# PacificBiosciences/aardvark

Hardware: NVIDIA B200
Metric: variant_clusters_per_sec (higher is better)
Workload: dtype int32

## Files before the change

### aardvark_b200/csrc/avk_lib.cu

```cuda
#include <cuda_runtime.h>

#include <algorithm>
#include <cstdio>
#include <cstdlib>
#include <cstring>
#include <string>
#include <chrono>
#include <thread>
#include <vector>

#include <cub/device/device_radix_sort.cuh>
#include <cub/device/device_scan.cuh>
#include <cub/device/device_select.cuh>
#include <thrust/iterator/counting_iterator.h>

#include "avk_solver.cuh"
#include "avk_thread_solver.cuh"
#include "avk_writers.h"
#include "avk_vcf.cuh"
#include "avk_inflate.cuh"

using namespace avk;

#define CK(call)                                                                                   \
    do {                                                                                           \
        cudaError_t e_ = (call);                                                                   \
        if (e_ != cudaSuccess) {                                                                   \
            ctx->err = std::string(#call) + ": " + cudaGetErrorString(e_);                         \
            return (e_ == cudaErrorMemoryAllocation) ? AVK_ERR_OOM : AVK_ERR_CUDA;                 \
        }                                                                                          \
    } while (0)


template <bool SMEM>
__device__ __forceinline__ void flush_work(typename Mem<SMEM>::addr hdr, unsigned long long *out) {
    typedef Mem<SMEM> M;
    if (lane_id() == 0 && out) {
        const u64 cells = LD64(hdr + WK_CELLS), matched = LD64(hdr + WK_MATCHED);
        const u32 al = LD32(hdr + WK_ALIGN), sp = LD32(hdr + WK_SPOPS), xp = LD32(hdr + WK_XPOPS);
        if (al) atomicAdd(out + 0, (unsigned long long)al);
        if (cells) atomicAdd(out + 1, (unsigned long long)cells);
        if (matched) atomicAdd(out + 2, (unsigned long long)matched);
        if (sp) atomicAdd(out + 3, (unsigned long long)sp);
        if (xp) atomicAdd(out + 4, (unsigned long long)xp);
    }
}
template <bool SMEM>
__device__ __forceinline__ void clear_work(typename Mem<SMEM>::addr hdr) {
    typedef Mem<SMEM> M;
    const int lane = lane_id();
    if (lane < 10) ST32(hdr + 8 + 4 * lane, 0);
    __syncwarp();
}

__device__ __forceinline__ VSeq<false> plain_seq(const u8 *p, int n) {
    VSeq<false> v;
    v.data = (u64)(uintptr_t)p; v.tail = v.data + (u64)n; v.mlen = n; v.len = n;
    return v;
}

__global__ void __launch_bounds__(256) k_alt_ed(DevBatch b, u64 v_base, u64 n_variants, u32 *alt_ed, u8 *scratch, int scratch_ints,
                                                unsigned long long *work_out) {
    const int lane = lane_id();
    const u64 warp = ((u64)blockIdx.x * blockDim.x + threadIdx.x) >> 5;
    const u64 n_warps = ((u64)gridDim.x * blockDim.x) >> 5;
    const u64 hdr = (u64)(uintptr_t)(scratch + warp * ((u64)scratch_ints * 4 + ARENA_HDR));
    clear_work<false>(hdr);
    for (u64 base = v_base + warp * 32; base < v_base + n_variants; base += n_warps * 32) {
        const u64 v = base + lane;
        bool coop = false;
        if (v < v_base + n_variants) {
            const u32 l0 = b.l0[v], l1 = b.l1[v];
            if (l0 == 1 && l1 == 1) alt_ed[v] = (b.pool[b.aoff[v]] != b.pool[b.aoff[v] + 1]) ? 1u : 0u;
            else coop = true;
        }
        unsigned m = __ballot_sync(AVK_FULL, coop);
        while (m) {
            const int src = __ffs(m) - 1;
            m &= m - 1;
            const u64 vv = base + src;
            const int l0 = (int)b.l0[vv], l1 = (int)b.l1[vv];
            const u8 *a0 = b.pool + b.aoff[vv];
            const u8 *a1 = a0 + l0;
            int ed;
            const int mn = min(l0, l1);
            if (mn == 0) ed = max(l0, l1);
            else if (2 * max(l0, l1) + 3 > scratch_ints) ed = 0;
            else {
                const int p = raw_lcp<false>((u64)(uintptr_t)a0, (u64)(uintptr_t)a1, mn);
                if (p == mn) ed = max(l0, l1) - mn;
                else {
                    ed = wfa_ed_warp<false>(plain_seq(a0, l0), plain_seq(a1, l1), hdr + ARENA_HDR, (scratch_ints - 3) / 2, hdr);
                    if (ed < 0) ed = 0;
                }
            }
            if (lane == 0) alt_ed[vv] = (u32)ed;
        }
    }
    flush_work<false>(hdr, work_out);
}

__global__ void __launch_bounds__(256) k_wfa_ed(const u32 *list, const u32 *n_list, const u8 *pool, const u64 *a_off, const u32 *a_len,
                                                const u64 *b_off, const u32 *b_len, u32 *ed_out, u8 *scratch,
                                                int scratch_ints, u32 *counter, unsigned long long *work_out) {
    const int lane = lane_id();
    const u64 warp = ((u64)blockIdx.x * blockDim.x + threadIdx.x) >> 5;
    const u64 hdr = (u64)(uintptr_t)(scratch + warp * ((u64)scratch_ints * 4 + ARENA_HDR));
    clear_work<false>(hdr);
    const u32 n_pairs = *n_list;
    for (;;) {
        u32 p = 0;
        if (lane == 0) p = atomicAdd(counter, 1u);
        p = __shfl_sync(AVK_FULL, p, 0);
        if (p >= n_pairs) break;
        p = list[p];
        const int ed = wfa_ed_warp<false>(plain_seq(pool + a_off[p], (int)a_len[p]), plain_seq(pool + b_off[p], (int)b_len[p]),
                                          hdr + ARENA_HDR, (scratch_ints - 3) / 2, hdr);
        if (lane == 0) ed_out[p] = (u32)ed;
    }
    flush_work<false>(hdr, work_out);
}

__global__ void __launch_bounds__(COOP_THREADS, 1) k_wfa_ed_cta(const u32 *list, const u32 *n_list, const u8 *pool, const u64 *a_off, const u32 *a_len,
                                                                const u64 *b_off, const u32 *b_len, u32 *ed_out, u8 *scratch, int scratch_ints,
                                                                int cap_ints, u32 *counter, unsigned long long *work_out) {
    __shared__ u32 s_idx;
    CoopJob &J = *(CoopJob *)avk_dyn_smem;
    const u64 hdr = (u64)(uintptr_t)(scratch + (u64)blockIdx.x * ((u64)scratch_ints * 4 + ARENA_HDR));
    if (threadIdx.x < 32) clear_work<false>(hdr);
    const u32 n = *n_list;
    for (;;) {
        __syncthreads();
        if (threadIdx.x == 0) s_idx = atomicAdd(counter, 1u);
        __syncthreads();
        const u32 idx = s_idx;
        if (idx >= n) break;
        const u32 p = list[idx];
        if (threadIdx.x == 0) {
            int *gw = (int *)(uintptr_t)(hdr + ARENA_HDR);
            gw[0] = 0;
            J.wf = hdr + ARENA_HDR;
            J.a_data = (u64)(uintptr_t)(pool + a_off[p]); J.a_mlen = J.a_len = (int)a_len[p]; J.a_tail = J.a_data + a_len[p];
            J.b_data = (u64)(uintptr_t)(pool + b_off[p]); J.b_mlen = J.b_len = (int)b_len[p]; J.b_tail = J.b_data + b_len[p];
            J.ed = 0; J.max_ed = 0x7ffffff0; J.to_full = 1; J.status = 0; J.exit_ = 0; J.matched = 0; J.cells = 0; J.cap_ints = cap_ints;
        }
        __threadfence();
        __syncthreads();
        coop_dwfa_body();
        int ed = J.ed;
        const int st = J.status;
        if (threadIdx.x < 32) {
            if (st == DWFA_COOP_SPILL) {
                const int rc = dwfa_run<false>(hdr + ARENA_HDR, &ed, (scratch_ints - 3) / 2, plain_seq(pool + a_off[p], (int)a_len[p]),
                                               plain_seq(pool + b_off[p], (int)b_len[p]), true, hdr);
                if (rc != DWFA_OK) ed = -1;
            }
            if (threadIdx.x == 0) {
                ed_out[p] = (u32)ed;
                *(u64 *)(uintptr_t)(hdr + WK_CELLS) += J.cells; *(u64 *)(uintptr_t)(hdr + WK_MATCHED) += J.matched; *(u32 *)(uintptr_t)(hdr + WK_ALIGN) += 1;
            }
        }
    }
    if (threadIdx.x < 32) flush_work<false>(hdr, work_out);
}

__global__ void __launch_bounds__(256) k_wfa_split(u64 n_pairs, const u32 *a_len, const u32 *b_len, u32 long_min, u32 max_sum, u32 *list_warp, u32 *n_warp,
                                                   u32 *list_cta, u32 *n_cta) {
    const u64 p = (u64)blockIdx.x * blockDim.x + threadIdx.x;
    if (p >= n_pairs) return;
    const u32 la = a_len[p], lb = b_len[p];
    const bool cta = min(la, lb) >= long_min && (u64)la + lb + 4096 <= max_sum && max(la, lb) < 60000u;
    if (cta) list_cta[atomicAdd(n_cta, 1u)] = (u32)p; else list_warp[atomicAdd(n_warp, 1u)] = (u32)p;
}

__global__ void __launch_bounds__(256) k_prep_size(DevBatch b, u64 n, u64 *sizes) {
    const u64 r = (u64)blockIdx.x * blockDim.x + threadIdx.x;
    if (r > n) return;
    if (r == n) { sizes[r] = 0; return; }
    const u64 v0 = b.var_off[r * 2], v1 = b.var_off[r * 2 + 2];
    u64 alle = 0;
    for (u64 v = v0; v < v1; ++v) alle += (u64)min(b.l0[v], 1u << 24) + (u64)min(b.l1[v], 1u << 24);
    sizes[r] = (PH_SIZE + VI_SIZE * (v1 - v0) + alle + 16 + 15) & ~15ull;
}

__global__ void __launch_bounds__(256) k_prep_fill(DevBatch b, u64 n_all, const u64 *offs, u8 *digest, const u32 *list, const u32 *n_list) {
    const int lane = lane_id();
    const u64 warp = ((u64)blockIdx.x * blockDim.x + threadIdx.x) >> 5;
    const u64 n_warps = ((u64)gridDim.x * blockDim.x) >> 5;
    const u64 n = list ? (u64)*n_list : n_all;
    for (u64 ri = warp; ri < n; ri += n_warps) {
        const u64 r = list ? (u64)list[ri] : ri;
        u8 *dig = digest + offs[r];
        int *hdr = (int *)dig;
        const long long start = b.start[r], end = b.end[r];
        const u64 v0[2] = {b.var_off[r * 2], b.var_off[r * 2 + 1]};
        const int cnt[2] = {(int)(b.var_off[r * 2 + 1] - v0[0]), (int)(b.var_off[r * 2 + 2] - v0[1])};
        const int N = cnt[0] + cnt[1];
        bool invalid = false;
        int s_l1 = 0, s_b0 = 0, s_al = 0, mx = (int)min(start, 0x7fffffffLL);
        for (int side = 0; side < 2; ++side) {
            for (int i = lane; i < cnt[side]; i += 32) {
                const u64 gv = v0[side] + i;
                const u32 l0 = b.l0[gv], l1 = b.l1[gv], p = b.pos[gv];
                invalid = invalid || l0 == 0 || l1 == 0 || b.vtype[gv] >= AVK_N_VARIANT_TYPES || b.zyg[gv] > AVK_ZYG_HOM_ALT;
                invalid = invalid || (long long)p < start || (long long)p + l0 > end;
                if (i > 0) invalid = invalid || b.pos[gv - 1] > p;
                s_l1 += (int)min(l1, 1u << 24);
                s_b0 += (int)min(max(l0, l1), 1u << 24);
                s_al += (int)min(l0, 1u << 24) + (int)min(l1, 1u << 24);
                mx = max(mx, (int)min(p + l0, 0x7fffffffu));
            }
        }
        invalid = __any_sync(AVK_FULL, invalid);
        s_l1 = __reduce_add_sync(AVK_FULL, s_l1); s_b0 = __reduce_add_sync(AVK_FULL, s_b0);
        s_al = __reduce_add_sync(AVK_FULL, s_al); mx = __reduce_max_sync(AVK_FULL, mx);
        if (invalid) {
            if (lane < PH_SIZE / 4) hdr[lane] = lane == 0 ? AVK_ST_BAD_INPUT : 0;
            continue;
        }
        u8 *recs = dig + PH_SIZE;
        for (int side = 0; side < 2; ++side) {
            const int nm = cnt[side], no = cnt[side ^ 1];
            const u64 vm = v0[side], vo = v0[side ^ 1];
            for (int i = lane; i < nm; i += 32) {
                const u64 gv = vm + i;
                const u32 p = b.pos[gv];
                int lo = 0, hi = no;
                while (lo < hi) {
                    const int m = (lo + hi) >> 1;
                    const u32 pm = b.pos[vo + m];
                    const bool before = side == 0 ? (pm < p) : (pm <= p);
                    if (before) lo = m + 1; else hi = m;
                }
                u32 *rec = (u32 *)(recs + (size_t)VI_SIZE * (i + lo));
                rec[VI_POS / 4] = p; rec[VI_L0 / 4] = b.l0[gv]; rec[VI_L1 / 4] = b.l1[gv]; rec[VI_AOFF / 4] = b.aoff[gv];
                rec[VI_ALTED / 4] = b.alt_ed[gv]; rec[VI_RAW / 4] = b.raw[gv]; rec[VI_GV / 4] = (u32)gv;
                rec[VI_FLAGS / 4] = (u32)b.vtype[gv] | ((u32)b.zyg[gv] << 8) | ((side == 0 ? 1u : 0u) << 16);
            }
        }
        __syncwarp();
        u8 *alle = recs + (size_t)VI_SIZE * N;
        u32 seen = 0;
        int acc = 0;
        for (int oi = 0; oi < N; ++oi) {
            u32 *rec = (u32 *)(recs + (size_t)VI_SIZE * oi);
            const int na = (int)(rec[VI_L0 / 4] + rec[VI_L1 / 4]);
            const u8 *src = b.pool + rec[VI_AOFF / 4];
            for (int i = lane; i < na; i += 32) alle[acc + i] = src[i];
            seen |= 1u << (rec[VI_FLAGS / 4] & 0xff);
            __syncwarp();
            if (lane == 0) rec[VI_AOFF / 4] = (u32)acc;
            acc += na;
        }
        __syncwarp();
        for (int oi = lane; oi < N; oi += 32) {
            u32 *rec = (u32 *)(recs + (size_t)VI_SIZE * oi);
            const u32 f = rec[VI_FLAGS / 4];
            rec[VI_FLAGS / 4] = f | ((u32)__popc(seen & ((1u << (f & 0xff)) - 1)) << 24);
        }
        if (lane == 0) {
            hdr[PH_STATUS / 4] = AVK_ST_OK; hdr[PH_N / 4] = N; hdr[PH_N0 / 4] = cnt[0]; hdr[PH_N1 / 4] = cnt[1];
            hdr[PH_SUM_L1 / 4] = s_l1; hdr[PH_B0 / 4] = s_b0; hdr[PH_SUM_ALLE / 4] = s_al; hdr[PH_MAX_END / 4] = mx;
            hdr[PH_NSLOTS / 4] = __popc(seen);
            int k = 0;
            for (int t = 0; t < AVK_N_VARIANT_TYPES; ++t) if (seen & (1u << t)) dig[PH_SLOT_TYPE + (k++)] = (u8)t;
        }
    }
}

enum { PREP_SMALL_N = 12 };
__global__ void __launch_bounds__(256) k_prep_fill_small(DevBatch b, u64 n, const u64 *offs, u8 *digest, u32 *big, u32 *big_ctr) {
    const u64 r = (u64)blockIdx.x * blockDim.x + threadIdx.x;
    if (r >= n) return;
    const u64 v0 = b.var_off[r * 2], vq = b.var_off[r * 2 + 1], v1 = b.var_off[r * 2 + 2];
    const int nT = (int)(vq - v0), nQ = (int)(v1 - vq), N = nT + nQ;
    if (N > PREP_SMALL_N) { big[atomicAdd(big_ctr, 1u)] = (u32)r; return; }
    u8 *dig = digest + offs[r];
    const long long start = b.start[r], end = b.end[r];
    bool invalid = false;
    int s_l1 = 0, s_b0 = 0, s_al = 0, mx = (int)min(start, 0x7fffffffLL);
    u32 seen = 0;
    for (u64 gv = v0; gv < v1; ++gv) {
        const u32 l0 = b.l0[gv], l1 = b.l1[gv], p = b.pos[gv], ty = b.vtype[gv];
        invalid = invalid || l0 == 0 || l1 == 0 || ty >= AVK_N_VARIANT_TYPES || b.zyg[gv] > AVK_ZYG_HOM_ALT;
        invalid = invalid || (long long)p < start || (long long)p + l0 > end;
        if (gv != v0 && gv != vq) invalid = invalid || b.pos[gv - 1] > p;
        s_l1 += (int)min(l1, 1u << 24); s_b0 += (int)min(max(l0, l1), 1u << 24); s_al += (int)min(l0, 1u << 24) + (int)min(l1, 1u << 24);
        mx = max(mx, (int)min(p + l0, 0x7fffffffu));
        seen |= 1u << (ty & 31u);
    }
    uint4 *h4 = (uint4 *)dig;
    if (invalid) {
        h4[0] = make_uint4((u32)AVK_ST_BAD_INPUT, 0, 0, 0); h4[1] = make_uint4(0, 0, 0, 0); h4[2] = make_uint4(0, 0, 0, 0); h4[3] = make_uint4(0, 0, 0, 0);
        return;
    }
    u8 *recs = dig + PH_SIZE, *alle = recs + (size_t)VI_SIZE * N;
    u64 it = v0, iq = vq;
    u32 acc = 0;
    for (int oi = 0; oi < N; ++oi) {
        const bool take_t = it < vq && (iq >= v1 || b.pos[it] <= b.pos[iq]);
        const u64 gv = take_t ? it : iq;
        if (take_t) ++it; else ++iq;
        const u32 l0 = b.l0[gv], l1 = b.l1[gv], ty = b.vtype[gv];
        uint4 *rec = (uint4 *)(recs + (size_t)VI_SIZE * oi);
        rec[0] = make_uint4(b.pos[gv], l0, l1, acc);
        rec[1] = make_uint4(b.alt_ed[gv], b.raw[gv], (u32)gv,
                            ty | ((u32)b.zyg[gv] << 8) | ((take_t ? 1u : 0u) << 16) | ((u32)__popc(seen & ((1u << ty) - 1)) << 24));
        const u8 *src = b.pool + b.aoff[gv];
        for (u32 k = 0; k < l0 + l1; ++k) alle[acc + k] = src[k];
        acc += l0 + l1;
    }
    h4[0] = make_uint4((u32)AVK_ST_OK, (u32)N, (u32)nT, (u32)nQ);
    h4[1] = make_uint4((u32)s_l1, (u32)s_b0, (u32)s_al, (u32)mx);
    u32 st[4] = {0, 0, 0, 0};
    int k = 0;
    for (int ty = 0; ty < AVK_N_VARIANT_TYPES; ++ty) if (seen & (1u << ty)) { st[k >> 2] |= (u32)ty << (8 * (k & 3)); ++k; }
    h4[2] = make_uint4((u32)__popc(seen), st[0], st[1], st[2]);
    h4[3] = make_uint4(0, 0, 0, 0);
}

__device__ __forceinline__ void zero_region_outputs(const DevBatch &b, const DevCompareOut &out, u64 r, bool metrics_only) {
    const int lane = lane_id();
    if (out.region_metrics) {
        u64 *gm = out.region_metrics + r * (u64)(AVK_N_GROUPS * AVK_N_METRICS);
        for (int i = lane; i < AVK_N_GROUPS * AVK_N_METRICS; i += 32) gm[i] = 0;
    }
    if (!metrics_only) {
        const u64 v0 = b.var_off[r * 2], v1 = b.var_off[r * 2 + 2];
        for (u64 v = v0 + lane; v < v1; v += 32) { out.vexp[v] = 0; out.vobs[v] = 0; out.vcls[v] = AVK_CLASS_UNKNOWN; }
        if (lane == 0) { out.ed1[r] = 0; out.ed2[r] = 0; out.type_mask[r] = 0; }
        if (out.seq_off && lane < 5) out.seq_len[r * 5 + lane] = 0;
    }
    __syncwarp();
}

__global__ void __launch_bounds__(256) k_compare_simple(DevBatch b, DevCompareOut out, avk_compare_cfg cfg, u64 n, u32 *work_list,
                                                        u32 *work_ctr, u32 *dense, u32 *dense_ctr, int dense_n, u64 *work_key) {
    const int lane = lane_id();
    const u64 warp = ((u64)blockIdx.x * blockDim.x + threadIdx.x) >> 5;
    const u64 n_warps = ((u64)gridDim.x * blockDim.x) >> 5;
    const bool enabled = !cfg.enable_exact_shortcut && !(out.seq_off && cfg.enable_sequences) && cfg.max_branch_factor >= 4;
    const u32 supported = (1u << AVK_VT_SNV) | (1u << AVK_VT_INSERTION) | (1u << AVK_VT_DELETION) | (1u << AVK_VT_INDEL) |
                          (1u << AVK_VT_TR_CONTRACTION) | (1u << AVK_VT_TR_EXPANSION) | (1u << AVK_VT_SV_DELETION) | (1u << AVK_VT_SV_INSERTION);
    for (u64 base = warp * 32; base < n; base += n_warps * 32) {
        const u64 r = base + lane;
        bool simple = false;
        int nvar = 0, npairs = 0;
        u32 gv[4] = {0, 0, 0, 0}, cp[2] = {0, 0}, vtype = 0;
        u64 s_c = 0, s_wT = 0, s_wQ = 0, s_X = 0, s_rT = 0, s_rQ = 0;
        if (r < n) {
            const u8 *dig = b.digest + b.digest_off[r];
            const int4 h = *(const int4 *)dig;
            const u32 c = b.contig[r];
            nvar = h.x == AVK_ST_OK ? h.y : 0;
            const int M = (h.y == 2 && h.z == 1 && h.w == 1) ? 1 : ((h.y == 4 && h.z == 2 && h.w == 2) ? 2 : 0);
            if (enabled && h.x == AVK_ST_OK && M && (M == 1 || cfg.max_branch_factor >= 16) && c < b.n_contigs && b.start[r] <= b.end[r] &&
                (u64)b.end[r] <= b.contig_len[c] && b.end[r] <= 0x7fff0000u) {
                const u8 *alle = dig + PH_SIZE + 2 * M * VI_SIZE;
                bool ok = true;
                u32 prev_pos = 0;
                for (int m = 0; m < M && ok; ++m) {
                    const u8 *rt = dig + PH_SIZE + 2 * m * VI_SIZE, *rq = rt + VI_SIZE;
                    const uint4 t0 = *(const uint4 *)rt, t1 = *(const uint4 *)(rt + 16), q0 = *(const uint4 *)rq, q1 = *(const uint4 *)(rq + 16);
                    const u32 zT = (t1.w >> 8) & 0xff, zQ = (q1.w >> 8) & 0xff;
                    const u32 cT = zT == AVK_ZYG_HOM_ALT ? 2u : (zT >= AVK_ZYG_UNPHASED_HET ? 1u : 0u);
                    const u32 cQ = zQ == AVK_ZYG_HOM_ALT ? 2u : (zQ >= AVK_ZYG_UNPHASED_HET ? 1u : 0u);
                    const u32 ty = t1.w & 0xffu;
                    ok = (t1.w & 0x10000u) && !(q1.w & 0x10000u) && ty == (q1.w & 0xffu) && ((supported >> ty) & 1u) && t0.x == q0.x &&
                         t0.y == q0.y && t0.z == q0.z && (t0.y == 1 || t0.z == 1) && t0.y + t0.z <= 64 && cT != 0 && cT == cQ;
                    if (M == 2) ok = ok && t0.y == 1 && t0.z == 1 && ty == AVK_VT_SNV && (m == 0 || t0.x > prev_pos);
                    if (!ok) break;
                    const u8 *aT = alle + t0.w + t0.y, *aQ = alle + q0.w + q0.y;
                    for (u32 k = 0; k < t0.z; ++k) ok = ok && aT[k] == aQ[k];
                    const bool anchored = aT[0] == b.contig_ptr[c][t0.x];
                    u32 X = 0;
                    if (t0.y == 1 && t0.z == 1) X = anchored ? 0u : 1u;
                    else if (anchored) X = (t0.y == 1 ? t0.z : t0.y) - 1u;
                    ok = ok && X != 0 && t1.y >= X && q1.y >= X;
                    gv[2 * m] = t1.z; gv[2 * m + 1] = q1.z; cp[m] = cT; vtype = ty; prev_pos = t0.x;
                    s_c += cT; s_wT += (u64)cT * t1.x; s_wQ += (u64)cT * q1.x; s_X += (u64)cT * X; s_rT += (u64)cT * t1.y; s_rQ += (u64)cT * q1.y;
                }
                simple = ok;
                npairs = M;
            }
        }
        const bool is_dense = r < n && !simple && nvar >= dense_n;
        const u32 rest = __ballot_sync(AVK_FULL, r < n && !simple && !is_dense);
        const u32 dn = __ballot_sync(AVK_FULL, is_dense);
        u32 pos0 = 0, pos1 = 0;
        if (lane == 0 && rest) pos0 = atomicAdd(work_ctr, (u32)__popc(rest));
        if (lane == 0 && dn) pos1 = atomicAdd(dense_ctr, (u32)__popc(dn));
        pos0 = __shfl_sync(AVK_FULL, pos0, 0);
        pos1 = __shfl_sync(AVK_FULL, pos1, 0);
        if (r < n && !simple && !is_dense) {
            const u32 slot_ = pos0 + __popc(rest & ((1u << lane) - 1));
            work_list[slot_] = (u32)r;
            if (work_key) {
                u64 key = 0;
                const int *dh = (const int *)(b.digest + b.digest_off[r]);
                const u32 edb = (u32)min(max(dh[PH_B0 / 4], 0), 16);
                const u32 wgt = (u32)max(nvar, 1) * (edb + 1u) * (edb + 1u);
                const u32 heavy = min(15u, (u32)(31 - __clz((int)max(wgt, 1u))));
                if (nvar > 0 && nvar <= 9) {
                    const u8 *recs = b.digest + b.digest_off[r] + PH_SIZE;
                    u32 prev = 0xffffffffu;
                    for (int oi = 0; oi < nvar; ++oi) {
                        const uint4 a = *(const uint4 *)(recs + (size_t)VI_SIZE * oi);
                        const u32 f = *(const u32 *)(recs + (size_t)VI_SIZE * oi + VI_FLAGS);
                        const u32 lc = (a.y == 1 && a.z == 1) ? 0u : (a.y == 1 ? 1u : (a.z == 1 ? 2u : 3u));
                        const u32 code = ((f >> 16) & 1u) | ((((f >> 8) & 0xffu) & 3u) << 1) | ((a.x == prev ? 1u : 0u) << 3) | (lc << 4);
                        key = (key << 6) | code;
                        prev = a.x;
                    }
                    key |= (u64)nvar << 54;
                } else key = (u64)min(nvar, 15) << 54;
                key |= (u64)(15u - heavy) << 58;
                work_key[slot_] = key;
            }
        }
        if (is_dense) dense[pos1 + __popc(dn & ((1u << lane) - 1))] = (u32)r;
        if (simple) {
            out.status[r] = AVK_ST_OK; out.ed1[r] = 0; out.ed2[r] = 0; out.type_mask[r] = (uint16_t)supported;
            for (int m = 0; m < npairs; ++m) {
                out.vexp[gv[2 * m]] = (u8)cp[m]; out.vobs[gv[2 * m]] = (u8)cp[m]; out.vcls[gv[2 * m]] = AVK_CLASS_TP;
                out.vexp[gv[2 * m + 1]] = (u8)cp[m]; out.vobs[gv[2 * m + 1]] = (u8)cp[m]; out.vcls[gv[2 * m + 1]] = AVK_CLASS_TP;
            }
        }
        if (out.tot_slots) {
            unsigned long long *slot = out.tot_slots + (size_t)(blockIdx.x & (TOT_SLOTS - 1)) * TOT_STRIDE;
            u32 left = __ballot_sync(AVK_FULL, simple);
            while (left) {
                const u32 ty = __shfl_sync(AVK_FULL, vtype, __ffs(left) - 1);
                const bool in = simple && vtype == ty;
                const u32 same = __ballot_sync(AVK_FULL, in);
                left &= ~same;
                unsigned long long v[7] = {(unsigned long long)npairs, (unsigned long long)s_c, (unsigned long long)s_wT, (unsigned long long)s_wQ,
                                           2ull * s_X, 2ull * s_rT, 2ull * s_rQ};
#pragma unroll
                for (int k = 0; k < 7; ++k) {
                    if (!in) v[k] = 0;
#pragma unroll
                    for (int o = 16; o; o >>= 1) v[k] += __shfl_xor_sync(AVK_FULL, v[k], o);
                }
                if (lane < 2) {
                    unsigned long long *g = slot + (lane == 0 ? 0 : (1 + ty) * AVK_N_METRICS);
                    atomicAdd(g + AVK_M_GT, v[0]); atomicAdd(g + AVK_M_GT + 2, v[0]);
                    atomicAdd(g + AVK_M_HAP, v[1]); atomicAdd(g + AVK_M_HAP + 2, v[1]);
                    atomicAdd(g + AVK_M_WEIGHTED_HAP, v[2]); atomicAdd(g + AVK_M_WEIGHTED_HAP + 2, v[3]);
                    atomicAdd(g + AVK_M_BASEPAIR, v[4]); atomicAdd(g + AVK_M_BASEPAIR + 2, v[4]);
                    atomicAdd(g + AVK_M_RECORD_BP, v[5]); atomicAdd(g + AVK_M_RECORD_BP + 2, v[6]);
                    if (lane == 0) { atomicAdd(slot + TOT_SOLVED, (unsigned long long)__popc(same)); atomicOr(slot + TOT_MASK, (unsigned long long)supported); }
                }
            }
        }
        u32 todo = out.region_metrics ? __ballot_sync(AVK_FULL, simple) : 0u;
        while (todo) {
            const int src = __ffs(todo) - 1;
            todo &= todo - 1;
            const u64 vM = (u64)__shfl_sync(AVK_FULL, npairs, src), vc = __shfl_sync(AVK_FULL, (unsigned long long)s_c, src);
            const u64 vwT = __shfl_sync(AVK_FULL, (unsigned long long)s_wT, src), vwQ = __shfl_sync(AVK_FULL, (unsigned long long)s_wQ, src);
            const u64 vrT = __shfl_sync(AVK_FULL, (unsigned long long)s_rT, src), vrQ = __shfl_sync(AVK_FULL, (unsigned long long)s_rQ, src);
            const u64 vX = __shfl_sync(AVK_FULL, (unsigned long long)s_X, src);
            const int grow = 1 + (int)__shfl_sync(AVK_FULL, vtype, src);
            u64 *dst = out.region_metrics + (base + src) * (u64)(AVK_N_GROUPS * AVK_N_METRICS);
#pragma unroll 1
            for (int i = lane; i < AVK_N_GROUPS * AVK_N_METRICS; i += 32) {
                const int g = i / AVK_N_METRICS, m = i - g * AVK_N_METRICS;
                u64 v = 0;
                if (g == 0 || g == grow) {
                    if (m == AVK_M_GT || m == AVK_M_GT + 2) v = vM;
                    else if (m == AVK_M_HAP || m == AVK_M_HAP + 2) v = vc;
                    else if (m == AVK_M_WEIGHTED_HAP) v = vwT;
                    else if (m == AVK_M_WEIGHTED_HAP + 2) v = vwQ;
                    else if (m == AVK_M_BASEPAIR || m == AVK_M_BASEPAIR + 2) v = 2 * vX;
                    else if (m == AVK_M_RECORD_BP) v = 2 * vrT;
                    else if (m == AVK_M_RECORD_BP + 2) v = 2 * vrQ;
                }
                dst[i] = v;
            }
        }
    }
}

__device__ __forceinline__ void count_error_block(const DevCompareOut &out) {
    if (out.tot_slots) atomicAdd(out.tot_slots + (size_t)(blockIdx.x & (TOT_SLOTS - 1)) * TOT_STRIDE + TOT_ERRORS, 1ull);
}

__global__ void __launch_bounds__(320) k_fold_slots(const unsigned long long *slots, unsigned long long *totals) {
    const int j = threadIdx.x;
    if (j >= TOT_COLS + 3) return;
    unsigned long long acc = 0;
    for (int s = 0; s < TOT_SLOTS; ++s) {
        const unsigned long long v = slots[(size_t)s * TOT_STRIDE + j];
        acc = (j == TOT_MASK) ? (acc | v) : (acc + v);
    }
    totals[j] = acc;
}

struct TierArgs {
    const u32 *work_list;
    const u32 *n_work_ptr;
    const u32 *work_list2;
    const u32 *n_work_ptr2;
    u32 *fail_list2;
    u32 *fail_ctr2;
    int dense_n;
    u32 n_work;
    u32 *work_ctr;
    u32 *fail_ctr;
    u8 *arena_base;
    long long arena_bytes;
    u32 *fail_list;
    int last_tier;
    unsigned long long *work_out;
    u8 *blobs;
    int wide_b0;
    u8 *spill_base;
    u32 spill_bytes;
    int n_lo, n_hi;
    int pop_budget;
    int batch_min;
    u8 *dense_blobs;
    u32 dense_cap;
};

enum { MODE_FUSED = 0, MODE_SEARCH = 1, MODE_SCORE = 2, MODE_COOP = 3 };

template <bool SMEM>
__device__ __forceinline__ RegionSolver<SMEM> &init_solver(const DevBatch &b, const TierArgs &t, DevBatch &sb, RegionSolver<SMEM> *sol) {
    typedef typename Mem<SMEM>::addr addr;
    if (threadIdx.x == 0) sb = b;
    __syncthreads();
    RegionSolver<SMEM> &s = sol[threadIdx.x >> 5];
    addr arena;
    if (SMEM) arena = (addr)((threadIdx.x >> 5) * (u32)t.arena_bytes);
    else arena = (addr)(uintptr_t)(t.arena_base + (((u64)blockIdx.x * blockDim.x + threadIdx.x) >> 5) * (u64)t.arena_bytes);
    if (lane_id() == 0) {
        s.bp = &sb;
        s.tma_phase = 0;
        s.tma_pending = 0;
        s.arena_bytes = (u32)t.arena_bytes;
        s.arena = arena;
        s.spill_base = nullptr; s.spill_bytes = 0; s.team = nullptr; s.pre_scored = 0;
        s.wide_b0 = t.wide_b0;
        if (SMEM && t.spill_base) {
            s.spill_base = t.spill_base + (((u64)blockIdx.x * blockDim.x + threadIdx.x) >> 5) * (u64)t.spill_bytes;
            s.spill_bytes = t.spill_bytes;
        }
        if (SMEM) mbar_init((u32)arena);
    }
    clear_work<SMEM>(arena);
    return s;
}

template <bool SMEM, int MIN_CTAS, int MODE>
__global__ void __launch_bounds__(256, MIN_CTAS) k_compare(DevBatch b, DevCompareOut out, avk_compare_cfg cfg, TierArgs t) {
    __shared__ DevBatch sb;
    __shared__ RegionSolver<SMEM> sol[8];
    const int lane = lane_id();
    RegionSolver<SMEM> &s = init_solver<SMEM>(b, t, sb, sol);
    const u32 n1 = t.n_work_ptr ? *t.n_work_ptr : t.n_work;
    const u32 n_work = n1 + (t.n_work_ptr2 ? *t.n_work_ptr2 : 0u);
    for (;;) {
        u32 idx = 0;
        if (lane == 0) idx = atomicAdd(t.work_ctr, 1u);
        idx = __shfl_sync(AVK_FULL, idx, 0);
        if (idx >= n_work) break;
        const u64 r = t.work_list ? (idx < n1 ? t.work_list[idx] : t.work_list2[idx - n1]) : idx;
        u8 *blob = t.blobs + r * (u64)RB_SIZE;
        int rc;
        if (MODE == MODE_SEARCH) {
            rc = s.compare_search_to_blob(r, cfg, blob);
            __syncwarp();
            if (rc == SOLVE_OK) continue;
            if (lane == 0) *(int *)(blob + RB_NRES) = (rc == SOLVE_WORKSPACE) ? RB_FUSED : RB_DONE;
        } else if (MODE == MODE_SCORE) {
            if (*(const int *)(blob + RB_NRES) <= 0) continue;
            rc = s.compare_score_from_blob(r, cfg, out, blob);
        } else {
            rc = s.solve_compare(r, cfg, out);
        }
        __syncwarp();
        if (rc == SOLVE_WORKSPACE) {
            if (!t.last_tier) {
                if (lane == 0) {
                    if (t.fail_list2 && s.N >= t.dense_n) t.fail_list2[atomicAdd(t.fail_ctr2, 1u)] = (u32)r;
                    else t.fail_list[atomicAdd(t.fail_ctr, 1u)] = (u32)r;
                }
                continue;
            }
            rc = AVK_ST_WORKSPACE;
        }
        if (rc != AVK_ST_OK) zero_region_outputs(sb, out, r, false);
        if (lane == 0) { out.status[r] = rc; if (rc != AVK_ST_OK) count_error_block(out); }
    }
    flush_work<SMEM>(s.arena, t.work_out);
}

__global__ void __launch_bounds__(COOP_THREADS, 1) k_compare_coop(DevBatch b, DevCompareOut out, avk_compare_cfg cfg, TierArgs t, int cap_ints) {
    __shared__ DevBatch sb;
    __shared__ RegionSolver<false> sol1;
    if (threadIdx.x == 0) { sb = b; ((CoopJob *)avk_dyn_smem)->cap_ints = cap_ints; ((CoopJob *)avk_dyn_smem)->exit_ = 0; }
    __syncthreads();
    if (threadIdx.x >= 32) { coop_helper_loop(); return; }
    const int lane = lane_id();
    RegionSolver<false> &s = sol1;
    const u64 arena = (u64)(uintptr_t)(t.arena_base + (u64)blockIdx.x * (u64)t.arena_bytes);
    if (lane == 0) {
        s.bp = &sb; s.tma_phase = 0; s.tma_pending = 0;
        s.arena_bytes = (u32)(t.arena_bytes > 0xfffffff0LL ? 0xfffffff0LL : t.arena_bytes); s.arena = arena;
        s.spill_base = nullptr; s.spill_bytes = 0; s.wide_b0 = 0; s.team = nullptr; s.pre_scored = 0;
    }
    clear_work<false>(arena);
    if (lane == 0) *(u32 *)(uintptr_t)(arena + WK_COOP) = 1u;
    __syncwarp();
    const u32 n_work = t.n_work_ptr ? *t.n_work_ptr : t.n_work;
    for (;;) {
        u32 idx = 0;
        if (lane == 0) idx = atomicAdd(t.work_ctr, 1u);
        idx = __shfl_sync(AVK_FULL, idx, 0);
        if (idx >= n_work) break;
        const u64 r = t.work_list ? t.work_list[idx] : idx;
        int rc = s.solve_compare(r, cfg, out);
        __syncwarp();
        if (rc == SOLVE_WORKSPACE) {
            if (!t.last_tier) {
                if (lane == 0) t.fail_list[atomicAdd(t.fail_ctr, 1u)] = (u32)r;
                continue;
            }
            rc = AVK_ST_WORKSPACE;
        }
        if (rc != AVK_ST_OK) zero_region_outputs(sb, out, r, false);
        if (lane == 0) { out.status[r] = rc; if (rc != AVK_ST_OK) count_error_block(out); }
// ... 339 lines not shown
                out.cls[r] = AVK_MERGE_DIFFERENT; out.n_idx[r] = 0;
                for (u32 k = 0; k < K; ++k) out.idx[r * K + k] = 0xFF;
            }
        }
    }
}

template <bool SMEM, int MIN_CTAS>
__global__ void __launch_bounds__(256, MIN_CTAS) k_merge_pairs(DevBatch b, avk_merge_cfg cfg, TierArgs t, MergeWork w) {
    __shared__ DevBatch sb;
    __shared__ RegionSolver<SMEM> sol[8];
    const int lane = lane_id();
    RegionSolver<SMEM> &s = init_solver<SMEM>(b, t, sb, sol);
    const u32 K = b.n_inputs;
    const u32 n_work = t.n_work_ptr ? *t.n_work_ptr : t.n_work;
    for (;;) {
        u32 idx = 0;
        if (lane == 0) idx = atomicAdd(t.work_ctr, 1u);
        idx = __shfl_sync(AVK_FULL, idx, 0);
        if (idx >= n_work) break;
        const u32 task = t.work_list ? t.work_list[idx] : idx;
        const u64 tk = w.tasks[task];
        const u64 r = tk >> 16;
        const u32 i = (u32)(tk >> 8) & 0xffu, j = (u32)tk & 0xffu;
        bool exact = false;
        int rc = s.merge_pair(r, i, j, cfg, &exact);
        __syncwarp();
        if (rc == SOLVE_WORKSPACE) {
            if (!t.last_tier) {
                if (lane == 0) t.fail_list[atomicAdd(t.fail_ctr, 1u)] = task;
                continue;
            }
            rc = AVK_ST_WORKSPACE;
        }
        if (lane == 0) {
            if (rc != AVK_ST_OK) atomicMin(w.pair_err + r, ((i * K - i * (i + 1) / 2 + (j - i - 1)) << 8) | (u32)rc);
            else if (exact) { atomicOr(w.rows + r * K + i, 1u << j); atomicOr(w.rows + r * K + j, 1u << i); }
        }
    }
    flush_work<SMEM>(s.arena, t.work_out);
}

__global__ void __launch_bounds__(256) k_merge_classify(DevBatch b, DevMergeOut out, avk_merge_cfg cfg, MergeWork w, u64 n) {
    __shared__ DevBatch sb;
    __shared__ RegionSolver<false> sol[8];
    const int lane = lane_id();
    if (threadIdx.x == 0) sb = b;
    __syncthreads();
    RegionSolver<false> &s = sol[threadIdx.x >> 5];
    if (lane == 0) s.bp = &sb;
    __syncwarp();
    const u32 K = b.n_inputs;
    const u64 warp = ((u64)blockIdx.x * blockDim.x + threadIdx.x) >> 5, n_warps = ((u64)gridDim.x * blockDim.x) >> 5;
    for (u64 r = warp; r < n; r += n_warps) {
        if (out.status[r] != AVK_ST_OK) continue;
        const int rc = s.merge_classify(r, cfg, out, w);
        __syncwarp();
        if (lane == 0 && rc != AVK_ST_OK) {
            out.status[r] = rc; out.cls[r] = AVK_MERGE_DIFFERENT; out.n_idx[r] = 0;
            for (u32 k = 0; k < K; ++k) out.idx[r * K + k] = 0xFF;
        }
    }
}

#define RED_COLS (AVK_N_GROUPS * AVK_N_METRICS)
__global__ void __launch_bounds__(288) k_reduce(u64 n, const int *status, const u64 *region_metrics, const uint16_t *type_mask,
                                                unsigned long long *totals, u32 *totals_mask, unsigned long long *solved,
                                                unsigned long long *errors, const u64 *strat_off, const u32 *strat_idx,
                                                const u64 *strat_mask, unsigned long long *strat_totals) {
    const int j = threadIdx.x;
    unsigned long long acc = 0, ok = 0, bad = 0;
    u32 mask = 0;
    for (u64 r0 = blockIdx.x; r0 < n; r0 += 4ull * gridDim.x) {
        bool good[4];
        unsigned long long v[4];
#pragma unroll
        for (int k = 0; k < 4; ++k) {
            const u64 r = r0 + (u64)k * gridDim.x;
            good[k] = r < n && status[r] == AVK_ST_OK;
        }
#pragma unroll
        for (int k = 0; k < 4; ++k) {
            const u64 r = r0 + (u64)k * gridDim.x;
            v[k] = (good[k] && j < RED_COLS) ? region_metrics[r * RED_COLS + j] : 0ull;
        }
#pragma unroll
        for (int k = 0; k < 4; ++k) {
            const u64 r = r0 + (u64)k * gridDim.x;
            if (r >= n) break;
            if (j == 0) { if (good[k]) { ok += 1; mask |= type_mask[r]; } else bad += 1; }
            acc += v[k];
            if (strat_off && v[k]) {
                for (u64 s = strat_off[r]; s < strat_off[r + 1]; ++s) atomicAdd(strat_totals + (u64)strat_idx[s] * RED_COLS + j, v[k]);
            } else if (strat_mask && v[k]) {
                for (u64 m = strat_mask[r]; m; m &= m - 1) atomicAdd(strat_totals + (u64)(__ffsll((long long)m) - 1) * RED_COLS + j, v[k]);
            }
        }
    }
    if (j < RED_COLS && acc) atomicAdd(totals + j, acc);
    if (j == 0) { atomicAdd(solved, ok); atomicAdd(errors, bad); atomicOr(totals_mask, mask); }
}

__global__ void __launch_bounds__(256) k_strat_contain(DevBatch b, u64 n, u32 n_strata, u32 n_contigs, const u64 *off, const u32 *first,
                                                       const u32 *pmax_last, u64 *mask_out) {
    const u64 r = (u64)blockIdx.x * blockDim.x + threadIdx.x;
    if (r >= n) return;
    const u64 t0 = b.var_off[r * 2], q0 = b.var_off[r * 2 + 1], q1 = b.var_off[r * 2 + 2];
    u64 start = ~0ull, end = 0;
    if (q0 > t0) { start = min(start, (u64)b.pos[t0]); end = max(end, (u64)b.pos[q0 - 1] + b.l0[q0 - 1]); }
    if (q1 > q0) { start = min(start, (u64)b.pos[q0]); end = max(end, (u64)b.pos[q1 - 1] + b.l0[q1 - 1]); }
    u64 mask = 0;
    const u32 c = b.contig[r];
    if (start < end && c < n_contigs) {
        const u64 a = start, z = end - 1;
        for (u32 s = 0; s < n_strata; ++s) {
            const u64 i0 = off[(u64)s * n_contigs + c], i1 = off[(u64)s * n_contigs + c + 1];
            u64 lo = i0, hi = i1;
            while (lo < hi) { const u64 m = (lo + hi) >> 1; if ((u64)first[m] <= a) lo = m + 1; else hi = m; }
            if (lo > i0 && (u64)pmax_last[lo - 1] >= z) mask |= 1ull << s;
        }
    }
    mask_out[r] = mask;
}

__global__ void __launch_bounds__(256) k_int_peak(int iters, int *sink) {
    int a0 = threadIdx.x, a1 = a0 + 1, a2 = a0 + 2, a3 = a0 + 3, a4 = a0 + 4, a5 = a0 + 5, a6 = a0 + 6, a7 = a0 + 7;
    const int k = blockIdx.x | 1;
#pragma unroll 4
    for (int i = 0; i < iters; ++i) {
        a0 = max(a0 + k, a1) ^ i; a1 = max(a1 + k, a2) ^ i; a2 = max(a2 + k, a3) ^ i; a3 = max(a3 + k, a4) ^ i;
        a4 = max(a4 + k, a5) ^ i; a5 = max(a5 + k, a6) ^ i; a6 = max(a6 + k, a7) ^ i; a7 = max(a7 + k, a0) ^ i;
    }
    if ((a0 ^ a1 ^ a2 ^ a3 ^ a4 ^ a5 ^ a6 ^ a7) == 0x7fffffff) sink[0] = a0;
}


struct DevBuf {
    void *p = nullptr;
    size_t cap = 0;
};

struct avk_ctx {
    int device = 0;
    cudaStream_t stream = nullptr;
    std::string err;
    uint64_t launches = 0;
    int sm_count = 148;
    std::vector<DevBuf> contig_bufs;
    std::vector<u64> contig_lens;
    DevBuf d_contig_ptr, d_contig_len;
    DevBuf region_id, contig, start, end, var_off, pos, vtype, zyg, raw, aoff, l0, l1, pool, alt_ed;
    DevBuf status, ed1, ed2, region_metrics, type_mask, vexp, vobs, vcls, totals, tot_slots, strat_off, strat_idx, strat_totals,
        seq_off, seq_len, seq_pool, m_cls, m_nidx, m_idx, m_rows, m_perr, m_tasks;
    DevBuf digest, digest_sizes, digest_offs, scan_tmp, blobs, scratch, arena, arena2, counters, fail_a, fail_b, fail_c, fail_d, fail_h, fail_w, fail_x, fail_t, fail_s, shape_key, work_ctr, pair_a_off, pair_b_off, pair_a_len, pair_b_len, pair_ed, pair_pool;
    DevBuf rb[24];
    DevBuf st_off, st_first, st_pmax, st_mask;
    u32 st_n = 0, st_contigs = 0;
    int dense_n = 0;
    bool have_batch = false;
    bool ids_resident = false;
    bool have_result = false, result_has_rows = false;
    u64 lo = 0, n_regions = 0, v_base = 0, n_variants = 0, p_base = 0, pool_bytes = 0;
    u64 seq_base = 0, strat_base = 0;
    u32 n_inputs = 0;
    u32 max_allele = 1;
    u64 pool_len = 0;
    u32 *h_pin = nullptr;
    cudaEvent_t ev[6] = {nullptr, nullptr, nullptr, nullptr, nullptr, nullptr};
    float last_ms[5] = {0, 0, 0, 0, 0};
    avk_work_counters last_work = {0, 0, 0, 0, 0, 0};
    u32 tier_fail[3] = {0, 0, 0};
    cudaEvent_t tev[4] = {nullptr, nullptr, nullptr, nullptr};
    cudaStream_t side[2] = {nullptr, nullptr};
    cudaEvent_t ev_fork = nullptr, ev_join[2] = {nullptr, nullptr}, dbg[3] = {nullptr, nullptr, nullptr};
    float tier_ms[3] = {0, 0, 0};
    long long coop_arena0 = 256LL << 20, coop_arena1 = 2048LL << 20;
    int coop_cap_ints = 26000;
    int wide_b0 = 256;
    DevBuf dense_blobs, dense_blobs2, spec_prof;
    bool use_spec_search = true;
    int thread_batch_min = 0;
    int thread_pop_budget = 0;
    bool use_thread_stage = true;
    bool sort_shapes = true;
    u64 thread_min_regions = 700000;
    avk_ctx *ref_owner = nullptr;
    avk_ctx *sib[2] = {nullptr, nullptr};
    int pipe_bins = 0;
    u64 pipe_min_regions = 1500000;
    u64 pipe_bin_regions = 1000000;
    cudaStream_t up = nullptr, dn = nullptr;
    cudaStream_t copy_streams[2] = {nullptr, nullptr};
    bool many_in_flight = false;
    u64 thread_min_regions_lanes = 100000;
    std::vector<avk_ctx *> lanes;
    int n_lanes = 0;
    u64 lane_min_regions = 2000000;
    cudaEvent_t ev_up = nullptr, ev_done = nullptr;
    bool own_streams = true;
};
static inline const avk_ctx *ref_of(const avk_ctx *ctx) { return ctx->ref_owner ? ctx->ref_owner : ctx; }

static int ensure(avk_ctx *ctx, DevBuf &b, size_t bytes) {
    if (bytes == 0) bytes = 16;
    if (b.cap >= bytes) return AVK_OK;
    if (b.p) { cudaFree(b.p); b.p = nullptr; b.cap = 0; }
    size_t want = bytes + bytes / 8 + 256;
    cudaError_t e = cudaMalloc(&b.p, want);
    if (e != cudaSuccess) {
        ctx->err = std::string("cudaMalloc(") + std::to_string(want) + "): " + cudaGetErrorString(e);
        cudaGetLastError();
        return AVK_ERR_OOM;
    }
    b.cap = want;
    return AVK_OK;
}
#define ENSURE(buf, bytes)                        \
    do {                                          \
        int rc_ = ensure(ctx, buf, (bytes));      \
        if (rc_ != AVK_OK) return rc_;            \
    } while (0)

static int upload(avk_ctx *ctx, DevBuf &b, const void *src, size_t bytes) {
    int rc = ensure(ctx, b, bytes);
    if (rc != AVK_OK) return rc;
    if (bytes) CK(cudaMemcpyAsync(b.p, src, bytes, cudaMemcpyHostToDevice, ctx->up ? ctx->up : ctx->stream));
    return AVK_OK;
}
static int uploads_done(avk_ctx *ctx) {
    if (ctx->up) {
        CK(cudaEventRecord(ctx->ev_up, ctx->up));
        CK(cudaStreamWaitEvent(ctx->stream, ctx->ev_up, 0));
    }
    return AVK_OK;
}
#define UPLOAD(buf, src, bytes)                          \
    do {                                                 \
        int rc_ = upload(ctx, buf, (src), (bytes));      \
        if (rc_ != AVK_OK) return rc_;                   \
    } while (0)

enum { COOP_CAP_INTS_MAX = 26000 };

static int configure_kernels(avk_ctx *ctx) {
    const int big = 222 * 1024;
#define SMEM_OPT_IN(k)                                                                            \
    do {                                                                                          \
        CK(cudaFuncSetAttribute(k, cudaFuncAttributeMaxDynamicSharedMemorySize, big));            \
        CK(cudaFuncSetAttribute(k, cudaFuncAttributePreferredSharedMemoryCarveout, 100));         \
    } while (0)
    SMEM_OPT_IN((k_compare<true, 3, MODE_SEARCH>));
    SMEM_OPT_IN((k_compare<true, 4, MODE_SCORE>));
    SMEM_OPT_IN((k_compare<true, 1, MODE_FUSED>));
    SMEM_OPT_IN(k_compare_team);
    SMEM_OPT_IN(k_compare_thread);
    SMEM_OPT_IN(k_search_spec);
    SMEM_OPT_IN(k_wfa_ed_cta);
    SMEM_OPT_IN((k_merge_pairs<true, 3>));
    SMEM_OPT_IN((k_merge_pairs<true, 1>));
#undef SMEM_OPT_IN
    CK(cudaFuncSetAttribute(k_compare_coop, cudaFuncAttributeMaxDynamicSharedMemorySize,
                            (int)(COOP_JOB_BYTES + 2 * sizeof(int) * (size_t)COOP_CAP_INTS_MAX)));
    return AVK_OK;
}

extern "C" int avk_create(int device, avk_ctx **out) {
    if (!out) return AVK_ERR_INVALID;
    *out = nullptr;
    int n = 0;
    if (cudaGetDeviceCount(&n) != cudaSuccess || device < 0 || device >= n) return AVK_ERR_CUDA;
    avk_ctx *ctx = new avk_ctx();
    ctx->device = device;
    if (cudaSetDevice(device) != cudaSuccess || cudaStreamCreateWithFlags(&ctx->stream, cudaStreamNonBlocking) != cudaSuccess) {
        delete ctx;
        return AVK_ERR_CUDA;
    }
    cudaDeviceProp prop;
    if (cudaGetDeviceProperties(&prop, device) == cudaSuccess) ctx->sm_count = prop.multiProcessorCount;
    if (configure_kernels(ctx) != AVK_OK) {
        fprintf(stderr, "[avk] avk_create: %s\n", ctx->err.c_str());
        cudaStreamDestroy(ctx->stream);
        delete ctx;
        return AVK_ERR_CUDA;
    }
    for (auto &e : ctx->ev) cudaEventCreate(&e);
    if (const char *dn = getenv("AVK_DENSE_N")) ctx->dense_n = std::max(3, atoi(dn));
    if (const char *s = getenv("AVK_TEST_COOP_ARENA_MB")) ctx->coop_arena0 = std::max(1LL, atoll(s)) << 20;
    if (const char *s = getenv("AVK_TEST_COOP_ARENA1_MB")) ctx->coop_arena1 = std::max(1LL, atoll(s)) << 20;
    if (const char *s = getenv("AVK_TEST_COOP_CAP_INTS")) ctx->coop_cap_ints = std::min<int>(COOP_CAP_INTS_MAX, std::max(64, atoi(s)));
    if (const char *s = getenv("AVK_TEST_WIDE_B0")) ctx->wide_b0 = std::max(1, atoi(s));
    if (const char *s = getenv("AVK_NO_THREAD_STAGE")) ctx->use_thread_stage = atoi(s) == 0;
    if (const char *s = getenv("AVK_NO_SPEC_SEARCH")) ctx->use_spec_search = atoi(s) == 0;
    if (const char *s = getenv("AVK_THREAD_POP_BUDGET")) ctx->thread_pop_budget = std::max(1, atoi(s));
    if (const char *s = getenv("AVK_THREAD_BATCH_MIN")) ctx->thread_batch_min = std::min(32, std::max(1, atoi(s)));
    { const int v = getenv("AVK_PACKED_DWFA") ? atoi(getenv("AVK_PACKED_DWFA")) : 0; cudaMemcpyToSymbol(g_avk_packed_dwfa, &v, sizeof(int)); }
    {
        unsigned long long *pp = nullptr;
        if (getenv("AVK_SPEC_PROFILE") && ensure(ctx, ctx->spec_prof, 65536 * 64) == AVK_OK) { pp = (unsigned long long *)ctx->spec_prof.p; cudaMemset(pp, 0, 65536 * 64); }
        cudaMemcpyToSymbol(g_spec_prof, &pp, sizeof(pp));
    }
    if (const char *s = getenv("AVK_NO_SHAPE_SORT")) ctx->sort_shapes = atoi(s) == 0;
    if (const char *s = getenv("AVK_THREAD_MIN_REGIONS")) ctx->thread_min_regions = ctx->thread_min_regions_lanes = (u64)std::max(0LL, atoll(s));
    if (const char *s = getenv("AVK_LANES")) ctx->n_lanes = std::max(0, std::min(8, atoi(s)));
    if (const char *s = getenv("AVK_LANE_MIN_REGIONS")) ctx->lane_min_regions = (u64)std::max(1LL, atoll(s));
    if (const char *s = getenv("AVK_PIPELINE_BINS")) ctx->pipe_bins = std::max(-1, atoi(s));
    if (const char *s = getenv("AVK_PIPELINE_BIN_REGIONS")) ctx->pipe_bin_regions = (u64)std::max(1LL, atoll(s));
    if (const char *s = getenv("AVK_PIPELINE_MIN_REGIONS")) ctx->pipe_min_regions = (u64)std::max(1LL, atoll(s));
    for (auto &e : ctx->tev) cudaEventCreate(&e);
    {
        int lo = 0, hi = 0;
        cudaDeviceGetStreamPriorityRange(&lo, &hi);
        for (auto &st : ctx->side) cudaStreamCreateWithPriority(&st, cudaStreamNonBlocking, lo);
    }
    cudaEventCreateWithFlags(&ctx->ev_fork, cudaEventDisableTiming);
    for (auto &e : ctx->ev_join) cudaEventCreateWithFlags(&e, cudaEventDisableTiming);
    for (auto &e : ctx->dbg) cudaEventCreate(&e);
    cudaEventCreateWithFlags(&ctx->ev_up, cudaEventDisableTiming);
    cudaEventCreateWithFlags(&ctx->ev_done, cudaEventDisableTiming);
    if (cudaMallocHost((void **)&ctx->h_pin, 4096) != cudaSuccess) { ctx->h_pin = nullptr; cudaGetLastError(); }
    if (!ctx->h_pin) { avk_destroy(ctx); return AVK_ERR_OOM; }
    memset(ctx->h_pin, 0, 4096);
    *out = ctx;
    return AVK_OK;
}

extern "C" int avk_create_lane(avk_ctx *owner, avk_ctx **out) {
    if (!owner || !out) return AVK_ERR_INVALID;
    if (owner->ref_owner) { owner->err = "avk_create_lane: the owner is itself a lane"; return AVK_ERR_INVALID; }
    const int rc = avk_create(owner->device, out);
    if (rc != AVK_OK) { owner->err = "avk_create_lane: could not create the context"; return rc; }
    (*out)->ref_owner = owner;
    (*out)->many_in_flight = owner->many_in_flight = true;
    return AVK_OK;
}

extern "C" void avk_destroy(avk_ctx *ctx) {
    if (!ctx) return;
    for (auto &sb : ctx->sib) if (sb) { avk_destroy(sb); sb = nullptr; }
    for (size_t i = 1; i < ctx->lanes.size(); ++i) avk_destroy(ctx->lanes[i]);
    ctx->lanes.clear();
    cudaSetDevice(ctx->device);
    cudaStreamSynchronize(ctx->stream);
    for (auto &st : ctx->side) if (st) cudaStreamSynchronize(st);
    for (cudaStream_t st : ctx->copy_streams) if (st) { cudaStreamSynchronize(st); cudaStreamDestroy(st); }
    DevBuf *bufs[] = {&ctx->d_contig_ptr, &ctx->d_contig_len, &ctx->region_id, &ctx->contig, &ctx->start, &ctx->end, &ctx->var_off,
                      &ctx->pos, &ctx->vtype, &ctx->zyg, &ctx->raw, &ctx->aoff, &ctx->l0, &ctx->l1, &ctx->pool, &ctx->alt_ed,
                      &ctx->status, &ctx->ed1, &ctx->ed2, &ctx->region_metrics, &ctx->type_mask, &ctx->vexp, &ctx->vobs, &ctx->vcls,
                      &ctx->totals, &ctx->tot_slots, &ctx->strat_off, &ctx->strat_idx, &ctx->strat_totals, &ctx->seq_off, &ctx->seq_len, &ctx->seq_pool,
                      &ctx->m_cls, &ctx->m_nidx, &ctx->m_idx, &ctx->m_rows, &ctx->m_perr, &ctx->m_tasks, &ctx->digest, &ctx->digest_sizes, &ctx->digest_offs, &ctx->scan_tmp, &ctx->blobs, &ctx->scratch, &ctx->arena, &ctx->arena2, &ctx->counters, &ctx->fail_a, &ctx->fail_b, &ctx->fail_c, &ctx->fail_d, &ctx->fail_h, &ctx->fail_w, &ctx->fail_x, &ctx->fail_t, &ctx->fail_s, &ctx->shape_key, &ctx->dense_blobs, &ctx->dense_blobs2, &ctx->spec_prof,
                      &ctx->work_ctr, &ctx->pair_a_off, &ctx->pair_b_off, &ctx->pair_a_len, &ctx->pair_b_len, &ctx->pair_ed, &ctx->pair_pool};
    for (DevBuf *b : bufs) if (b->p) cudaFree(b->p);
    for (DevBuf &b : ctx->rb) if (b.p) cudaFree(b.p);
    for (DevBuf *b : {&ctx->st_off, &ctx->st_first, &ctx->st_pmax, &ctx->st_mask}) if (b->p) cudaFree(b->p);
    for (DevBuf &b : ctx->contig_bufs) if (b.p) cudaFree(b.p);
    for (auto &e : ctx->ev) if (e) cudaEventDestroy(e);
    for (auto &e : ctx->tev) if (e) cudaEventDestroy(e);
    for (auto &e : ctx->ev_join) if (e) cudaEventDestroy(e);
    for (auto &e : ctx->dbg) if (e) cudaEventDestroy(e);
    if (ctx->ev_fork) cudaEventDestroy(ctx->ev_fork);
    if (ctx->ev_up) cudaEventDestroy(ctx->ev_up);
    if (ctx->ev_done) cudaEventDestroy(ctx->ev_done);
    if (ctx->own_streams) {
        for (auto &st : ctx->side) if (st) cudaStreamDestroy(st);
        cudaStreamDestroy(ctx->stream);
    }
    if (ctx->h_pin) cudaFreeHost(ctx->h_pin);
    delete ctx;
}

extern "C" const char *avk_last_error(const avk_ctx *ctx) { return ctx ? ctx->err.c_str() : "null context"; }
extern "C" uint64_t avk_launch_count(const avk_ctx *ctx) {
    if (!ctx) return 0;
    uint64_t n = ctx->launches;
    for (const avk_ctx *sb : ctx->sib) if (sb) n += sb->launches;
    for (size_t i = 1; i < ctx->lanes.size(); ++i) n += ctx->lanes[i]->launches;
    return n;
}

extern "C" int avk_set_reference(avk_ctx *ctx, uint32_t n_contigs, const uint8_t *const *seqs, const uint64_t *lens) {
    if (ctx && ctx->ref_owner) { ctx->err = "a lane reads its owner's reference: call avk_set_reference on the owner"; return AVK_ERR_INVALID; }
    if (!ctx || (n_contigs && (!seqs || !lens))) return AVK_ERR_INVALID;
    CK(cudaSetDevice(ctx->device));
    for (DevBuf &b : ctx->contig_bufs) if (b.p) cudaFree(b.p);
    ctx->contig_bufs.assign(n_contigs, DevBuf());
    ctx->contig_lens.assign(lens, lens + n_contigs);
    std::vector<const u8 *> ptrs(n_contigs);
    for (uint32_t c = 0; c < n_contigs; ++c) {
        ENSURE(ctx->contig_bufs[c], lens[c] + 64);
        if (lens[c]) CK(cudaMemcpyAsync(ctx->contig_bufs[c].p, seqs[c], lens[c], cudaMemcpyHostToDevice, ctx->stream));
        ptrs[c] = (const u8 *)ctx->contig_bufs[c].p;
    }
    UPLOAD(ctx->d_contig_ptr, ptrs.data(), sizeof(u8 *) * n_contigs);
    UPLOAD(ctx->d_contig_len, lens, sizeof(u64) * n_contigs);
    CK(cudaStreamSynchronize(ctx->stream));
    ctx->have_result = false;
    return AVK_OK;
}

extern "C" int avk_set_stratifications(avk_ctx *ctx, const avk_strat_intervals *in) {
    if (ctx && ctx->ref_owner) { ctx->err = "a lane reads its owner's stratifications: call avk_set_stratifications on the owner"; return AVK_ERR_INVALID; }
    if (!ctx) return AVK_ERR_INVALID;
    if (!in || in->n_strata > 64 || (in->n_strata && in->n_contigs && !in->off)) { ctx->err = "avk_set_stratifications: at most 64 strata, non-null offsets"; return AVK_ERR_INVALID; }
    CK(cudaSetDevice(ctx->device));
    const u64 cells = (u64)in->n_strata * in->n_contigs;
    const u64 n_iv = cells ? in->off[cells] : 0;
    if (n_iv && (!in->first || !in->last)) { ctx->err = "avk_set_stratifications: null interval arrays"; return AVK_ERR_INVALID; }
    std::vector<u32> first(n_iv), pmax(n_iv);
    std::vector<std::pair<u32, u32>> iv;
    for (u64 k = 0; k < cells; ++k) {
        const u64 i0 = in->off[k], i1 = in->off[k + 1];
        if (i0 > i1 || i1 > n_iv) { ctx->err = "avk_set_stratifications: offsets are not monotone"; return AVK_ERR_INVALID; }
        iv.clear();
        for (u64 i = i0; i < i1; ++i) iv.emplace_back(in->first[i], in->last[i]);
        std::sort(iv.begin(), iv.end());
        u32 run = 0;
        for (u64 i = i0; i < i1; ++i) { run = std::max(run, iv[i - i0].second); first[i] = iv[i - i0].first; pmax[i] = run; }
    }
    std::vector<u64> off(cells + 1, 0);
    for (u64 k = 0; k <= cells && cells; ++k) off[k] = in->off[k];
    UPLOAD(ctx->st_off, off.data(), 8 * (cells + 1));
    UPLOAD(ctx->st_first, first.data(), 4 * n_iv);
    UPLOAD(ctx->st_pmax, pmax.data(), 4 * n_iv);
    CK(cudaStreamSynchronize(ctx->stream));
    ctx->st_n = in->n_strata; ctx->st_contigs = in->n_contigs;
    for (auto &sb : ctx->sib) if (sb) { const int rc = avk_set_stratifications(sb, in); if (rc != AVK_OK) return rc; }
    return AVK_OK;
}

struct BinScan {
    u64 lo = 0, hi = 0, v0 = 0, v1 = 0, p0 = 0, p1 = 0, sum_alle = 0;
    u32 max_allele = 1;
};

static int bin_range(avk_ctx *ctx, const avk_region_batch *b, u64 lo, u64 hi, BinScan &sc) {
    const u64 K = b->n_inputs;
    const avk_variant_table &t = b->variants;
    sc.lo = lo; sc.hi = hi;
    if (hi == lo) return AVK_OK;
    const u64 *vo = b->var_off;
    sc.v0 = vo[lo * K]; sc.v1 = vo[hi * K];
    if (sc.v0 > sc.v1 || sc.v1 > t.n_variants) { ctx->err = "var_off outside the variant table"; return AVK_ERR_INVALID; }
    if (sc.v1 > sc.v0 && (!t.position || !t.variant_type || !t.zygosity || !t.raw_allele_space || !t.allele_off || !t.a0_len || !t.a1_len || !t.allele_pool)) {
        ctx->err = "null variant arrays";
        return AVK_ERR_INVALID;
    }
    return AVK_OK;
}
static int scan_bin(avk_ctx *ctx, const avk_region_batch *b, BinScan &sc) {
    const u64 K = b->n_inputs, lo = sc.lo, hi = sc.hi;
    const avk_variant_table &t = b->variants;
    if (hi == lo) return AVK_OK;
    const u64 *vo = b->var_off;
    const u64 nv = sc.v1 - sc.v0, nr = (hi - lo) * K;
    const int nt = (int)std::min<u64>(12, std::max<u64>(1, (nv + nr) / 400000));
    struct Part { u64 p0 = ~0ull, p1 = 0, sum = 0; u32 mx = 1; int bad = 0; };
    std::vector<Part> parts(nt);
    auto work = [&](int ti) {
        Part &P = parts[ti];
        for (u64 i = lo * K + nr * ti / nt, e = lo * K + nr * (ti + 1) / nt; i < e; ++i) if (vo[i] > vo[i + 1]) P.bad = 1;
        const u64 pool_len = t.allele_pool_len;
        for (u64 v = sc.v0 + nv * ti / nt, e = sc.v0 + nv * (ti + 1) / nt; v < e; ++v) {
            const u64 a = t.allele_off[v], l0 = t.a0_len[v], l1 = t.a1_len[v];
            if (l0 > (1u << 24) || l1 > (1u << 24)) { P.bad = 2; continue; }
            if (a + l0 + l1 > pool_len) { P.bad = 3; continue; }
            P.p0 = std::min(P.p0, a); P.p1 = std::max(P.p1, a + l0 + l1);
            P.sum += l0 + l1;
            P.mx = std::max(P.mx, (u32)std::max(l0, l1));
        }
    };
    if (nt == 1) work(0);
    else {
        std::vector<std::thread> th;
        for (int ti = 0; ti < nt; ++ti) th.emplace_back(work, ti);
        for (auto &x : th) x.join();
    }
    u64 p0 = ~0ull, p1 = 0;
    for (const Part &P : parts) {
        if (P.bad) {
            ctx->err = P.bad == 1 ? "var_off is not monotone" : (P.bad == 2 ? "allele longer than 16 MiB" : "allele range outside the allele pool");
            return AVK_ERR_INVALID;
        }
        p0 = std::min(p0, P.p0); p1 = std::max(p1, P.p1);
        sc.sum_alle += P.sum; sc.max_allele = std::max(sc.max_allele, P.mx);
    }
    if (p1 > p0) { sc.p0 = p0; sc.p1 = p1; }
    return AVK_OK;
}

static int validate_batch(avk_ctx *ctx, const avk_region_batch *b, bool compare) {
    if (!b) { ctx->err = "null batch"; return AVK_ERR_INVALID; }
    if (compare ? b->n_inputs != 2 : (b->n_inputs < 1 || b->n_inputs > 32)) { ctx->err = "unsupported n_inputs"; return AVK_ERR_INVALID; }
    if (b->n_regions >= (1ull << 32) - 1 || b->variants.n_variants >= (1ull << 32) || b->variants.allele_pool_len >= (1ull << 32)) {
        ctx->err = "batch too large for 32-bit indices; split it";
        return AVK_ERR_INVALID;
    }
    if (b->n_regions && (!b->region_id || !b->contig || !b->start || !b->end || !b->var_off)) { ctx->err = "null region arrays"; return AVK_ERR_INVALID; }
    if (b->n_regions && b->var_off[b->n_regions * b->n_inputs] != b->variants.n_variants) { ctx->err = "var_off does not cover the variant table"; return AVK_ERR_INVALID; }
    return AVK_OK;
}

static int upload_batch(avk_ctx *ctx, const avk_region_batch *b, BinScan &sc) {
    if (ref_of(ctx)->contig_bufs.empty()) { ctx->err = "avk_set_reference has not been called"; return AVK_ERR_NO_REFERENCE; }
    const u64 lo = sc.lo, n = sc.hi - sc.lo, K = b->n_inputs, v0 = sc.v0, nv = sc.v1 - sc.v0;
    const avk_variant_table &t = b->variants;
    ctx->have_batch = false; ctx->have_result = false; ctx->ids_resident = false;
    UPLOAD(ctx->contig, b->contig + lo, 4 * n);
    UPLOAD(ctx->start, b->start + lo, 4 * n);
    UPLOAD(ctx->end, b->end + lo, 4 * n);
    if (n) UPLOAD(ctx->var_off, b->var_off + lo * K, 8 * (n * K + 1));
    else { ENSURE(ctx->var_off, 8); CK(cudaMemsetAsync(ctx->var_off.p, 0, 8, ctx->stream)); }
    UPLOAD(ctx->pos, t.position + v0, 4 * nv);
    UPLOAD(ctx->vtype, t.variant_type + v0, nv);
    UPLOAD(ctx->zyg, t.zygosity + v0, nv);
    UPLOAD(ctx->raw, t.raw_allele_space + v0, 4 * nv);
    UPLOAD(ctx->aoff, t.allele_off + v0, 4 * nv);
    UPLOAD(ctx->l0, t.a0_len + v0, 4 * nv);
    UPLOAD(ctx->l1, t.a1_len + v0, 4 * nv);
    ENSURE(ctx->alt_ed, 4 * nv);
    int rc = scan_bin(ctx, b, sc);
    if (rc != AVK_OK) { cudaStreamSynchronize(ctx->up ? ctx->up : ctx->stream); return rc; }
    UPLOAD(ctx->pool, t.allele_pool + sc.p0, sc.p1 - sc.p0);
    ctx->max_allele = sc.max_allele;
    ctx->pool_len = sc.sum_alle;
    ctx->lo = lo; ctx->n_regions = n; ctx->v_base = v0; ctx->n_variants = nv; ctx->p_base = sc.p0; ctx->pool_bytes = sc.p1 - sc.p0;
    ctx->n_inputs = b->n_inputs;
    ctx->have_batch = true;
    return AVK_OK;
}

template <class T>
static inline T *biased(const DevBuf &b, u64 base) { return (T *)((uintptr_t)b.p - (uintptr_t)(base * sizeof(T))); }

static DevBatch dev_batch(avk_ctx *ctx) {
    DevBatch d;
    const u64 vb = ctx->v_base;
    d.n_regions = ctx->n_regions; d.n_inputs = ctx->n_inputs;
    d.region_id = nullptr; d.contig = (const u32 *)ctx->contig.p;
    d.start = (const u32 *)ctx->start.p; d.end = (const u32 *)ctx->end.p; d.var_off = (const u64 *)ctx->var_off.p;
    d.pos = biased<const u32>(ctx->pos, vb); d.vtype = biased<const u8>(ctx->vtype, vb); d.zyg = biased<const u8>(ctx->zyg, vb);
    d.raw = biased<const u32>(ctx->raw, vb); d.aoff = biased<const u32>(ctx->aoff, vb); d.l0 = biased<const u32>(ctx->l0, vb);
    d.l1 = biased<const u32>(ctx->l1, vb);
    d.pool = biased<const u8>(ctx->pool, ctx->p_base);
    d.contig_ptr = (const u8 *const *)ref_of(ctx)->d_contig_ptr.p; d.contig_len = (const u64 *)ref_of(ctx)->d_contig_len.p;
    d.n_contigs = (u32)ref_of(ctx)->contig_lens.size();
    d.alt_ed = biased<const u32>(ctx->alt_ed, vb);
    d.digest = (const u8 *)ctx->digest.p;
    d.digest_off = (const u64 *)ctx->digest_offs.p;
    return d;
}

static int run_alt_ed(avk_ctx *ctx, const DevBatch &db) {
    if (ctx->n_variants == 0) return AVK_OK;
    const int blocks = ctx->sm_count * 4, threads = 256;
    const int warps = blocks * threads / 32;
    const int scratch_ints = (2 * (int)ctx->max_allele + 8 + 3) / 4 * 4;
    ENSURE(ctx->scratch, (size_t)warps * ((size_t)scratch_ints * 4 + ARENA_HDR));
    k_alt_ed<<<blocks, threads, 0, ctx->stream>>>(db, ctx->v_base, ctx->n_variants, biased<u32>(ctx->alt_ed, ctx->v_base), (u8 *)ctx->scratch.p,
                                                   scratch_ints, (unsigned long long *)ctx->work_ctr.p);
    ctx->launches += 1;
    CK(cudaGetLastError());
    return AVK_OK;
}

struct Stage {
    int mode;
    bool smem;
    int min_ctas;
    long long arena_bytes;
    int ctas;
    int warps;
    int in_list;
    int in_ctr;
    int work_ctr;
    int fail_list;
    int fail_ctr;
    int stream;
    int n_lo, n_hi;
};

template <class P, class F>
static int run_stages(avk_ctx *ctx, u64 n, const std::vector<Stage> &stages, P pre, int first_ctr, F launch) {
    if (n == 0) return AVK_OK;
    const int sm = ctx->sm_count;
    ENSURE(ctx->fail_a, 4 * n);
    ENSURE(ctx->fail_b, 4 * n);
    ENSURE(ctx->counters, 256);
    u32 *ctrs = (u32 *)ctx->counters.p;
    CK(cudaMemsetAsync(ctrs, 0, 256, ctx->stream));
    u32 *fail_lists[2] = {(u32 *)ctx->fail_a.p, (u32 *)ctx->fail_b.p};
    size_t garena = 0;
    for (const Stage &st : stages) if (!st.smem) garena = std::max(garena, (size_t)st.ctas * st.warps * (size_t)st.arena_bytes);
    if (garena) ENSURE(ctx->arena, garena);
    ENSURE(ctx->arena2, (size_t)sm * 8 * (size_t)(1u << 20));
    CK(cudaEventRecord(ctx->tev[0], ctx->stream));
    pre(ctrs);
    int ev = 1;
    for (size_t i = 0; i < stages.size(); ++i) {
        const Stage &st = stages[i];
        TierArgs a = {};
        a.work_list = st.in_list < 0 ? nullptr : fail_lists[st.in_list];
        a.n_work_ptr = st.in_list < 0 ? (first_ctr >= 0 ? ctrs + first_ctr : nullptr) : ctrs + st.in_ctr;
        a.n_work = (u32)n;
        a.work_ctr = ctrs + st.work_ctr;
        a.fail_ctr = ctrs + st.fail_ctr;
        a.arena_base = (u8 *)ctx->arena.p;
        a.arena_bytes = st.arena_bytes;
        a.fail_list = fail_lists[st.fail_list];
        a.last_tier = 0;
        a.work_out = (unsigned long long *)ctx->work_ctr.p;
        a.blobs = (u8 *)ctx->blobs.p;
        a.spill_base = nullptr; a.spill_bytes = 0;
        if (st.smem && st.arena_bytes >= 16384) { a.spill_base = (u8 *)ctx->arena2.p; a.spill_bytes = 1u << 20; }
        a.n_lo = st.n_lo; a.n_hi = st.n_hi;
        int ctas = st.ctas;
        if (st.in_list < 0) ctas = (int)std::min<u64>((u64)ctas, (n + st.warps - 1) / st.warps);
        launch(st, a, ctas, ctx->stream);
        ctx->launches += 1;
        CK(cudaGetLastError());
        if (ev < 3 && (i + 1 < stages.size())) CK(cudaEventRecord(ctx->tev[ev++], ctx->stream));
    }
    while (ev < 4) CK(cudaEventRecord(ctx->tev[ev++], ctx->stream));
    const Stage &lastst = stages.back();
    CK(cudaMemcpyAsync(ctx->h_pin, ctrs, 64, cudaMemcpyDeviceToHost, ctx->stream));
    CK(cudaStreamSynchronize(ctx->stream));
    const u32 *host_ctrs = ctx->h_pin;
    for (int t = 0; t < 3; ++t) cudaEventElapsedTime(&ctx->tier_ms[t], ctx->tev[t], ctx->tev[t + 1]);
    {
        int k = 0;
        for (const Stage &st : stages) if (k < 3) ctx->tier_fail[k++] = host_ctrs[st.fail_ctr];
        while (k < 3) ctx->tier_fail[k++] = 0;
    }
    u32 n_work = host_ctrs[lastst.fail_ctr];
    int cur_list = lastst.fail_list;
    const Stage big[2] = {{MODE_FUSED, false, 1, 64LL << 20, (sm + 7) / 8, 8, 0, 0, 0, 0, 0, 0, 0, 0x7fffffff}, {MODE_FUSED, false, 1, 2048LL << 20, 1, 8, 0, 0, 0, 0, 0, 0, 0, 0x7fffffff}};
    for (int t = 0; t < 2 && n_work > 0; ++t) {
        ENSURE(ctx->arena, (size_t)big[t].ctas * big[t].warps * (size_t)big[t].arena_bytes);
        CK(cudaMemsetAsync(ctrs + 32, 0, 8, ctx->stream));
        TierArgs a = {};
        a.work_list = fail_lists[cur_list];
        a.n_work_ptr = nullptr;
        a.n_work = n_work;
        a.work_ctr = ctrs + 32;
        a.fail_ctr = ctrs + 33;
        a.arena_base = (u8 *)ctx->arena.p;
        a.arena_bytes = big[t].arena_bytes;
        a.fail_list = fail_lists[cur_list ^ 1];
        a.last_tier = t == 1;
        a.work_out = (unsigned long long *)ctx->work_ctr.p;
        a.blobs = (u8 *)ctx->blobs.p;
        a.n_lo = 0; a.n_hi = 0x7fffffff;
        launch(big[t], a, big[t].ctas, ctx->stream);
        ctx->launches += 1;
        CK(cudaGetLastError());
        CK(cudaMemcpyAsync(ctx->h_pin, ctrs + 32, 8, cudaMemcpyDeviceToHost, ctx->stream));
        CK(cudaStreamSynchronize(ctx->stream));
        n_work = ctx->h_pin[1];
        cur_list ^= 1;
    }
    return AVK_OK;
}

template <bool SMEM, int MIN_CTAS, int MODE>
static void launch_compare(const DevBatch &db, const DevCompareOut &out, const avk_compare_cfg &c, const TierArgs &a, int ctas, int warps, cudaStream_t strm) {
    const size_t smem = SMEM ? (size_t)a.arena_bytes * warps : 0;
    k_compare<SMEM, MIN_CTAS, MODE><<<ctas, 32 * warps, smem, strm>>>(db, out, c, a);
}
template <bool SMEM, int MIN_CTAS>
static void launch_merge_pairs(const DevBatch &db, const avk_merge_cfg &c, const TierArgs &a, const MergeWork &w, int ctas, int warps, cudaStream_t strm) {
    const size_t smem = SMEM ? (size_t)a.arena_bytes * warps : 0;
    k_merge_pairs<SMEM, MIN_CTAS><<<ctas, 32 * warps, smem, strm>>>(db, c, a, w);
}

static int run_prepare(avk_ctx *ctx, const DevBatch &db) {
    const u64 n = ctx->n_regions;
    if (n == 0) return AVK_OK;
    u64 *sizes = (u64 *)ctx->digest_sizes.p, *offs = (u64 *)ctx->digest_offs.p;
    k_prep_size<<<(unsigned)((n + 1 + 255) / 256), 256, 0, ctx->stream>>>(db, n, sizes);
    size_t tmp_bytes = 0;
    cub::DeviceScan::ExclusiveSum(nullptr, tmp_bytes, sizes, offs, (int)(n + 1), ctx->stream);
    ENSURE(ctx->scan_tmp, tmp_bytes);
    cub::DeviceScan::ExclusiveSum(ctx->scan_tmp.p, tmp_bytes, sizes, offs, (int)(n + 1), ctx->stream);
    ENSURE(ctx->fail_a, 4 * n);
    ENSURE(ctx->counters, 256);
    u32 *big_ctr = (u32 *)ctx->counters.p + 40;
    CK(cudaMemsetAsync(big_ctr, 0, 4, ctx->stream));
    k_prep_fill_small<<<(unsigned)((n + 255) / 256), 256, 0, ctx->stream>>>(db, n, offs, (u8 *)ctx->digest.p, (u32 *)ctx->fail_a.p, big_ctr);
    k_prep_fill<<<ctx->sm_count * 2, 256, 0, ctx->stream>>>(db, n, offs, (u8 *)ctx->digest.p, (const u32 *)ctx->fail_a.p, big_ctr);
    ctx->launches += 4;
    CK(cudaGetLastError());
    return AVK_OK;
}

static inline bool strata_wanted(const avk_compare_out *out) { return out->strat_totals && out->n_strata; }

struct CompareRun {
    DevBatch db;
    DevCompareOut out;
    avk_compare_cfg cfg;
    bool strata = false;
    const u64 *strat_off = nullptr;
    const u32 *strat_idx = nullptr;
    const u64 *strat_mask = nullptr;
    bool want_contain = false;
    u32 n_strata = 0;
};

static void launch_stage(avk_ctx *ctx, const CompareRun &R, const Stage &st, const TierArgs &a, int ctas, cudaStream_t strm) {
    if (st.mode == MODE_COOP) {
        const size_t smem = COOP_JOB_BYTES + 2 * sizeof(int) * (size_t)ctx->coop_cap_ints;
        k_compare_coop<<<ctas, COOP_THREADS, smem, strm>>>(R.db, R.out, R.cfg, a, ctx->coop_cap_ints);
    }
    else if (st.mode == MODE_SEARCH) launch_compare<true, 3, MODE_SEARCH>(R.db, R.out, R.cfg, a, ctas, st.warps, strm);
    else if (st.mode == MODE_SCORE) launch_compare<true, 4, MODE_SCORE>(R.db, R.out, R.cfg, a, ctas, st.warps, strm);
    else if (st.smem) launch_compare<true, 1, MODE_FUSED>(R.db, R.out, R.cfg, a, ctas, st.warps, strm);
    else launch_compare<false, 1, MODE_FUSED>(R.db, R.out, R.cfg, a, ctas, st.warps, strm);
}

static TierArgs tier_args(avk_ctx *ctx, const u32 *list, int in_ctr, int work_ctr, u32 *fail_list, int fail_ctr, long long arena_bytes, u8 *garena) {
    u32 *ctrs = (u32 *)ctx->counters.p;
    TierArgs a = {};
    a.work_list = list; a.n_work_ptr = list ? ctrs + in_ctr : nullptr; a.n_work = (u32)ctx->n_regions;
    a.work_ctr = ctrs + work_ctr; a.fail_ctr = ctrs + fail_ctr; a.fail_list = fail_list;
    a.arena_base = garena; a.arena_bytes = arena_bytes; a.last_tier = 0;
    a.work_out = (unsigned long long *)ctx->work_ctr.p; a.blobs = (u8 *)ctx->blobs.p; a.n_lo = 0; a.n_hi = 0x7fffffff;
    a.spill_base = nullptr; a.spill_bytes = 0;
    return a;
}

static int run_compare_pipeline(avk_ctx *ctx, const CompareRun &R) {
    const u64 n = ctx->n_regions;
    if (n == 0) return AVK_OK;
    const int sm = ctx->sm_count;
    ENSURE(ctx->fail_a, 4 * n); ENSURE(ctx->fail_b, 4 * n); ENSURE(ctx->fail_c, 4 * n); ENSURE(ctx->fail_d, 4 * n); ENSURE(ctx->fail_h, 4 * n); ENSURE(ctx->fail_w, 4 * n); ENSURE(ctx->fail_x, 4 * n); ENSURE(ctx->fail_t, 4 * n);
    ENSURE(ctx->counters, 256);
    ENSURE(ctx->blobs, (size_t)n * RB_SIZE);
    u32 *ctrs = (u32 *)ctx->counters.p;
    u32 *LA = (u32 *)ctx->fail_a.p, *LB = (u32 *)ctx->fail_b.p, *LD = (u32 *)ctx->fail_d.p;
    CK(cudaMemsetAsync(ctrs, 0, 256, ctx->stream));
    ENSURE(ctx->arena, (size_t)sm * 8 * (size_t)(2LL << 20));
    ENSURE(ctx->arena2, 2 * (size_t)sm * 8 * (size_t)(1u << 20));
    const Stage SEARCH = {MODE_SEARCH, true, 3, 8192, sm * 3, 8}, SCORE = {MODE_SCORE, true, 4, 5120, sm * 4, 8};
    const Stage S1 = {MODE_FUSED, true, 1, 27648, sm, 8}, G0 = {MODE_FUSED, false, 1, 2LL << 20, sm, 8};
    CK(cudaEventRecord(ctx->tev[0], ctx->stream));
    u32 *LW = (u32 *)ctx->fail_h.p, *LA2 = (u32 *)ctx->fail_w.p, *LX = (u32 *)ctx->fail_x.p;
    const bool thread_stage = ctx->use_thread_stage && n >= (ctx->many_in_flight ? ctx->thread_min_regions_lanes : ctx->thread_min_regions);
    const int dense_n = ctx->dense_n ? ctx->dense_n : (thread_stage ? 10 : (n >= 250000 ? 8 : 6));
    u64 *keys = nullptr;
    if (thread_stage && ctx->sort_shapes) {
        ENSURE(ctx->shape_key, 16 * n);
        ENSURE(ctx->fail_s, 4 * n);
        keys = (u64 *)ctx->shape_key.p;
        CK(cudaMemsetAsync(keys, 0xff, 8 * n, ctx->stream));
    }
    k_compare_simple<<<sm * 8, 256, 0, ctx->stream>>>(R.db, R.out, R.cfg, n, LW, ctrs + 12, LX, ctrs + 17, dense_n, keys);
    if (keys) {
        size_t need = 0;
        cub::DeviceRadixSort::SortPairs(nullptr, need, keys, keys + n, LW, (u32 *)ctx->fail_s.p, (int)n, 0, 64, ctx->stream);
        ENSURE(ctx->scan_tmp, need);
        cub::DeviceRadixSort::SortPairs(ctx->scan_tmp.p, need, keys, keys + n, LW, (u32 *)ctx->fail_s.p, (int)n, 0, 64, ctx->stream);
        ctx->launches += 1;
    }
    const size_t spill_warp = 1u << 20, spill_half = (size_t)sm * 8 * spill_warp;
    const u32 dense_cap = (u32)std::min<u64>(n, std::max<u64>(65536, n / 16));
    auto spec_then_team = [&](const u32 *list, int in_ctr, int spec_ctr, int team_ctr, DevBuf &blobs, u8 *spill, cudaStream_t strm) -> int {
        TierArgs a = tier_args(ctx, list, in_ctr, team_ctr, LB, 5, 108 * 1024, nullptr);
        a.spill_base = spill; a.spill_bytes = (u32)spill_warp;
        if (ctx->use_spec_search) {
            ENSURE(blobs, (size_t)dense_cap * avk_sp::SPB_SIZE);
            TierArgs sa = tier_args(ctx, list, in_ctr, spec_ctr, nullptr, 21, 0, nullptr);
            sa.dense_blobs = (u8 *)blobs.p; sa.dense_cap = dense_cap;
            k_search_spec<<<sm, 32 * SPEC_WARPS, SPEC_WARPS * (sizeof(avk_sp::Shared) + 32 * sizeof(avk_sp::Scratch)), strm>>>(R.db, R.out, R.cfg, sa);
            ctx->launches += 1;
            a.dense_blobs = sa.dense_blobs; a.dense_cap = dense_cap;
        }
        k_compare_team<<<sm, 128 * TEAMS_PER_CTA, TEAMS_PER_CTA * (size_t)a.arena_bytes, strm>>>(R.db, R.out, R.cfg, a);
        ctx->launches += 1;
        return AVK_OK;
    };
    CK(cudaEventRecord(ctx->ev_fork, ctx->stream));
    CK(cudaStreamWaitEvent(ctx->side[0], ctx->ev_fork, 0));
    {
        const int rc = spec_then_team(LX, 17, 20, 4, ctx->dense_blobs, (u8 *)ctx->arena2.p, ctx->stream);
        if (rc != AVK_OK) return rc;
    }
    CK(cudaEventRecord(ctx->tev[1], ctx->stream));
    if (thread_stage) {
        u32 *LW2 = (u32 *)ctx->fail_t.p;
        TierArgs a = tier_args(ctx, keys ? (const u32 *)ctx->fail_s.p : LW, 12, 19, LW2, 13, sizeof(avk_ts::Work), nullptr);
        a.batch_min = ctx->thread_batch_min;
        a.pop_budget = ctx->thread_pop_budget ? ctx->thread_pop_budget : (n >= 2500000 ? 64 : (n >= 1200000 ? 48 : 32));
        k_compare_thread<<<(unsigned)std::min<u64>((u64)sm, (n + THREAD_TPB - 1) / THREAD_TPB), THREAD_TPB, THREAD_TPB * sizeof(avk_ts::Work), ctx->side[0]>>>(R.db, R.out, R.cfg, a);
        ctx->launches += 1;
        const int rc = spec_then_team(LW2, 13, 22, 23, ctx->dense_blobs2, (u8 *)ctx->arena2.p + spill_half, ctx->side[0]);
        if (rc != AVK_OK) return rc;
    } else {
        const int small_ctas = (int)std::min<u64>((u64)SEARCH.ctas, (n + 7) / 8);
        launch_stage(ctx, R, SEARCH, tier_args(ctx, LW, 12, 0, LA, 1, SEARCH.arena_bytes, nullptr), small_ctas, ctx->side[0]);
        launch_stage(ctx, R, SCORE, tier_args(ctx, LW, 12, 2, LA2, 15, SCORE.arena_bytes, nullptr), (int)std::min<u64>((u64)SCORE.ctas, (n + 7) / 8), ctx->side[0]);
        ctx->launches += 2;
        const int rc = spec_then_team(LA, 1, 22, 23, ctx->dense_blobs2, (u8 *)ctx->arena2.p + spill_half, ctx->side[0]);
        if (rc != AVK_OK) return rc;
    }
    CK(cudaEventRecord(ctx->ev_join[0], ctx->side[0]));
    CK(cudaStreamWaitEvent(ctx->stream, ctx->ev_join[0], 0));
    CK(cudaEventRecord(ctx->tev[2], ctx->stream));
    {
        TierArgs a = tier_args(ctx, LA2, 15, 16, LB, 5, S1.arena_bytes, nullptr);
        a.spill_base = (u8 *)ctx->arena2.p; a.spill_bytes = 1u << 20;
        launch_stage(ctx, R, S1, a, S1.ctas, ctx->stream);
    }
    {
        TierArgs a = tier_args(ctx, LB, 5, 9, LD, 7, G0.arena_bytes, (u8 *)ctx->arena.p);
        a.wide_b0 = ctx->wide_b0;
        launch_stage(ctx, R, G0, a, G0.ctas, ctx->stream);
    }
    CK(cudaEventRecord(ctx->tev[3], ctx->stream));
    ctx->launches += 3;
    CK(cudaGetLastError());
    return AVK_OK;
}

static int run_big_tiers(avk_ctx *ctx, const CompareRun &R, u32 n_work) {
    const int sm = ctx->sm_count;
    u32 *ctrs = (u32 *)ctx->counters.p;
    Stage big[2] = {{MODE_COOP, false, 1, ctx->coop_arena0, sm, 1}, {MODE_COOP, false, 1, ctx->coop_arena1, 16, 1}};
    const u32 *cur = (u32 *)ctx->fail_d.p;
    u32 *other = (u32 *)ctx->fail_c.p;
    for (int t = 0; t < 2 && n_work > 0; ++t) {
        big[t].ctas = (int)std::min<u64>((u64)big[t].ctas, n_work);
        if (n_work > 1 && n_work <= 4096) { k_sort_biggest_first<<<1, 1024, 0, ctx->stream>>>(R.db, (u32 *)cur, n_work); ctx->launches += 1; }
        ENSURE(ctx->arena, (size_t)big[t].ctas * big[t].warps * (size_t)big[t].arena_bytes);
        CK(cudaMemsetAsync(ctrs + 32, 0, 8, ctx->stream));
        if (getenv("AVK_DEBUG")) cudaEventRecord(ctx->dbg[0], ctx->stream);
        TierArgs a = tier_args(ctx, cur, 0, 32, other, 33, big[t].arena_bytes, (u8 *)ctx->arena.p);
        a.n_work_ptr = nullptr; a.n_work = n_work; a.last_tier = t == 1;
        launch_stage(ctx, R, big[t], a, big[t].ctas, ctx->stream);
        ctx->launches += 1;
        CK(cudaGetLastError());
        CK(cudaMemcpyAsync(ctx->h_pin + 64, ctrs + 32, 8, cudaMemcpyDeviceToHost, ctx->stream));
        CK(cudaStreamSynchronize(ctx->stream));
        if (getenv("AVK_DEBUG")) {
            float ms = 0;
            cudaEventRecord(ctx->dbg[1], ctx->stream); cudaEventSynchronize(ctx->dbg[1]); cudaEventElapsedTime(&ms, ctx->dbg[0], ctx->dbg[1]);
            fprintf(stderr, "[avk] big tier %d (cooperative, %lld MB): %u clusters in, %u rejected, %.1f ms\n", t, big[t].arena_bytes >> 20, n_work, ctx->h_pin[65], ms);
        }
        n_work = ctx->h_pin[65];
        const u32 *tmp = cur; cur = other; other = (u32 *)tmp;
    }
    return AVK_OK;
}

static int run_finalize(avk_ctx *ctx, const CompareRun &R) {
    const u64 n = ctx->n_regions;
    unsigned long long *tot = (unsigned long long *)ctx->totals.p;
    if (!R.strata) {
        k_fold_slots<<<1, 320, 0, ctx->stream>>>((const unsigned long long *)ctx->tot_slots.p, tot);
        ctx->launches += 1;
    } else {
        CK(cudaMemsetAsync(tot, 0, 8 * RED_COLS + 64, ctx->stream));
        CK(cudaMemsetAsync(ctx->strat_totals.p, 0, 8ull * RED_COLS * R.n_strata, ctx->stream));
        if (n) {
            k_reduce<<<(unsigned)std::min<u64>(n, (u64)ctx->sm_count * 8), 288, 0, ctx->stream>>>(
                n, R.out.status, R.out.region_metrics, R.out.type_mask, tot, (u32 *)(tot + RED_COLS), tot + RED_COLS + 1, tot + RED_COLS + 2,
                R.strat_off, R.strat_idx, R.strat_mask, (unsigned long long *)ctx->strat_totals.p);
            ctx->launches += 1;
        }
    }
    CK(cudaGetLastError());
    return AVK_OK;
}

static int queue_counter_copies(avk_ctx *ctx) {
    CK(cudaMemcpyAsync(ctx->h_pin, ctx->counters.p, 128, cudaMemcpyDeviceToHost, ctx->stream));
    CK(cudaMemcpyAsync(ctx->h_pin + 128, ctx->work_ctr.p, 40, cudaMemcpyDeviceToHost, ctx->stream));
    CK(cudaEventRecord(ctx->ev_done, ctx->stream));
    return AVK_OK;
}

static int compare_launch(avk_ctx *ctx, const avk_compare_cfg *cfg, bool want_seq, bool want_rows, bool strata, u32 n_strata, bool strat_dev, bool want_contain, CompareRun &R) {
    const u64 n = ctx->n_regions, nv = ctx->n_variants;
    const bool rows = want_rows || strata;
    if (strat_dev || want_contain) ENSURE(ctx->st_mask, 8 * n);
    ENSURE(ctx->status, 4 * n); ENSURE(ctx->ed1, 4 * n); ENSURE(ctx->ed2, 4 * n);
    if (rows) ENSURE(ctx->region_metrics, 8ull * RED_COLS * n);
    ENSURE(ctx->type_mask, 2 * n);
    ENSURE(ctx->vexp, nv); ENSURE(ctx->vobs, nv); ENSURE(ctx->vcls, nv);
    ENSURE(ctx->totals, 8 * RED_COLS + 64);
    ENSURE(ctx->tot_slots, 8ull * TOT_SLOTS * TOT_STRIDE);
    ENSURE(ctx->counters, 256);
    ENSURE(ctx->work_ctr, 64);
    if (strata) ENSURE(ctx->strat_totals, 8ull * RED_COLS * n_strata);
    CK(cudaMemsetAsync(ctx->work_ctr.p, 0, 64, ctx->stream));
    CK(cudaMemsetAsync(ctx->tot_slots.p, 0, 8ull * TOT_SLOTS * TOT_STRIDE, ctx->stream));
    ENSURE(ctx->digest, (size_t)n * (PH_SIZE + 32) + (size_t)VI_SIZE * nv + (size_t)ctx->pool_len + 256);
    ENSURE(ctx->digest_sizes, 8 * (n + 1));
    ENSURE(ctx->digest_offs, 8 * (n + 1));
    R.db = dev_batch(ctx);
    DevCompareOut &out = R.out;
    out.status = (int *)ctx->status.p; out.ed1 = (u32 *)ctx->ed1.p; out.ed2 = (u32 *)ctx->ed2.p;
    out.region_metrics = rows ? (u64 *)ctx->region_metrics.p : nullptr;
    out.tot_slots = strata ? nullptr : (unsigned long long *)ctx->tot_slots.p;
    out.type_mask = (uint16_t *)ctx->type_mask.p;
    out.vexp = biased<u8>(ctx->vexp, ctx->v_base); out.vobs = biased<u8>(ctx->vobs, ctx->v_base); out.vcls = biased<u8>(ctx->vcls, ctx->v_base);
    out.seq_off = want_seq ? (const u64 *)ctx->seq_off.p : nullptr;
    out.seq_len = (u32 *)ctx->seq_len.p; out.seq_pool = biased<u8>(ctx->seq_pool, ctx->seq_base);
    R.cfg = *cfg;
    R.strata = strata; R.n_strata = n_strata;
    R.strat_off = (strata && !strat_dev) ? (const u64 *)ctx->strat_off.p : nullptr;
    R.strat_idx = (strata && !strat_dev) ? biased<const u32>(ctx->strat_idx, ctx->strat_base) : nullptr;
    R.strat_mask = (strata && strat_dev) ? (const u64 *)ctx->st_mask.p : nullptr;
    R.want_contain = strat_dev || want_contain;
    ctx->have_result = false;

    CK(cudaEventRecord(ctx->ev[0], ctx->stream));
    int rc = run_alt_ed(ctx, R.db);
    if (rc != AVK_OK) return rc;
    rc = run_prepare(ctx, R.db);
    if (rc != AVK_OK) return rc;
    CK(cudaEventRecord(ctx->ev[1], ctx->stream));
    if (R.want_contain && n) {
        const avk_ctx *so = ref_of(ctx);
        k_strat_contain<<<(unsigned)((n + 255) / 256), 256, 0, ctx->stream>>>(R.db, n, so->st_n, so->st_contigs, (const u64 *)so->st_off.p,
                                                                              (const u32 *)so->st_first.p, (const u32 *)so->st_pmax.p, (u64 *)ctx->st_mask.p);
        ctx->launches += 1;
    }
    rc = run_compare_pipeline(ctx, R);
    if (rc != AVK_OK) return rc;
    CK(cudaEventRecord(ctx->ev[2], ctx->stream));
    CK(cudaEventRecord(ctx->ev[3], ctx->stream));
    rc = run_finalize(ctx, R);
    if (rc != AVK_OK) return rc;
    CK(cudaEventRecord(ctx->ev[4], ctx->stream));
    ctx->result_has_rows = rows;
    return queue_counter_copies(ctx);
}

static int compare_finish(avk_ctx *ctx, const CompareRun &R, bool *redo) {
    if (redo) *redo = false;
    CK(cudaEventSynchronize(ctx->ev_done));
    const u32 *h = ctx->h_pin;
    if (ctx->n_regions) {
        for (int t = 0; t < 3; ++t) cudaEventElapsedTime(&ctx->tier_ms[t], ctx->tev[t], ctx->tev[t + 1]);
        ctx->tier_fail[0] = h[1]; ctx->tier_fail[1] = h[5]; ctx->tier_fail[2] = h[7];
        if (h[7] > 0) {
            int rc = run_big_tiers(ctx, R, h[7]);
            if (rc != AVK_OK) return rc;
            CK(cudaEventRecord(ctx->ev[2], ctx->stream));
            CK(cudaEventRecord(ctx->ev[3], ctx->stream));
            rc = run_finalize(ctx, R);
            if (rc != AVK_OK) return rc;
            CK(cudaEventRecord(ctx->ev[4], ctx->stream));
            rc = queue_counter_copies(ctx);
            if (rc != AVK_OK) return rc;
            CK(cudaEventSynchronize(ctx->ev_done));
            if (redo) *redo = true;
        }
    } else {
        for (int t = 0; t < 3; ++t) { ctx->tier_ms[t] = 0; ctx->tier_fail[t] = 0; }
    }
    ctx->have_result = true;
    return AVK_OK;
}

static int fetch_timings(avk_ctx *ctx) {
    CK(cudaEventSynchronize(ctx->ev[4]));
    cudaEventElapsedTime(&ctx->last_ms[0], ctx->ev[0], ctx->ev[1]);
    cudaEventElapsedTime(&ctx->last_ms[1], ctx->ev[1], ctx->ev[2]);
    cudaEventElapsedTime(&ctx->last_ms[2], ctx->ev[2], ctx->ev[3]);
    cudaEventElapsedTime(&ctx->last_ms[3], ctx->ev[3], ctx->ev[4]);
    cudaEventElapsedTime(&ctx->last_ms[4], ctx->ev[0], ctx->ev[4]);
    CK(cudaEventSynchronize(ctx->ev_done));
    const unsigned long long *w = (const unsigned long long *)(ctx->h_pin + 128);
    ctx->last_work.alignments = w[0]; ctx->last_work.cells = w[1]; ctx->last_work.matched_bases = w[2];
    ctx->last_work.search_pops = w[3]; ctx->last_work.exact_pops = w[4];
    return AVK_OK;
}

#define DL(dst, buf, bytes)                                                                                     \
    do {                                                                                                        \
        if ((dst) && (bytes)) CK(cudaMemcpyAsync((dst), (buf).p, (bytes), cudaMemcpyDeviceToHost, ds)); \
    } while (0)

struct BinTotals {
    unsigned long long tot[RED_COLS + 8];
    std::vector<u64> strat;
};

static int download_compare_async(avk_ctx *ctx, avk_compare_out *out, bool want_seq, u64 seq_bytes) {
    const u64 n = ctx->n_regions, nv = ctx->n_variants, lo = ctx->lo, vb = ctx->v_base;
    const cudaStream_t ds = ctx->dn ? ctx->dn : ctx->stream;
    if (ctx->dn) CK(cudaStreamWaitEvent(ctx->dn, ctx->ev_done, 0));
    DL(out->status ? out->status + lo : nullptr, ctx->status, 4 * n);
    DL(out->ed1 ? out->ed1 + lo : nullptr, ctx->ed1, 4 * n);
    DL(out->ed2 ? out->ed2 + lo : nullptr, ctx->ed2, 4 * n);
    if (out->region_metrics && n) {
        if (!ctx->result_has_rows) { ctx->err = "per-region metric rows were not kept by this run (AVK_CMP_KEEP_REGION_ROWS)"; return AVK_ERR_INVALID; }
        DL(out->region_metrics + lo * RED_COLS, ctx->region_metrics, 8ull * RED_COLS * n);
    }
    DL(out->type_mask ? out->type_mask + lo : nullptr, ctx->type_mask, 2 * n);
    DL(out->var_expected ? out->var_expected + vb : nullptr, ctx->vexp, nv);
    DL(out->var_observed ? out->var_observed + vb : nullptr, ctx->vobs, nv);
    DL(out->var_class ? out->var_class + vb : nullptr, ctx->vcls, nv);
    CK(cudaMemcpyAsync(ctx->h_pin + 256, ctx->totals.p, 8 * RED_COLS + 64, cudaMemcpyDeviceToHost, ds));
    if (out->containment && ctx->st_mask.p) DL(out->containment + lo, ctx->st_mask, 8 * n);
    if (want_seq) {
        DL(out->seq_len + lo * 5, ctx->seq_len, 4 * 5 * n);
        DL(out->seq_pool + ctx->seq_base, ctx->seq_pool, seq_bytes);
    }
    return AVK_OK;
}

static int collect_totals(avk_ctx *ctx, const avk_compare_out *out, bool strata, BinTotals &bt) {
    memcpy(bt.tot, ctx->h_pin + 256, 8 * RED_COLS + 64);
    bt.strat.clear();
    if (strata) {
        bt.strat.resize((size_t)RED_COLS * out->n_strata);
        const cudaStream_t ds = ctx->dn ? ctx->dn : ctx->stream;
        CK(cudaMemcpyAsync(bt.strat.data(), ctx->strat_totals.p, 8ull * RED_COLS * out->n_strata, cudaMemcpyDeviceToHost, ds));
        CK(cudaStreamSynchronize(ds));
    }
    return AVK_OK;
}

static void store_totals(avk_compare_out *out, const BinTotals &bt, bool strata, bool accumulate) {
    if (out->totals) for (int j = 0; j < RED_COLS; ++j) out->totals[j] = (accumulate ? out->totals[j] : 0) + bt.tot[j];
    if (out->totals_mask) *out->totals_mask = (uint16_t)((accumulate ? *out->totals_mask : 0) | (bt.tot[RED_COLS] & 0xffff));
    if (out->solved_blocks) *out->solved_blocks = (accumulate ? *out->solved_blocks : 0) + bt.tot[RED_COLS + 1];
    if (out->error_blocks) *out->error_blocks = (accumulate ? *out->error_blocks : 0) + bt.tot[RED_COLS + 2];
    if (strata && out->strat_totals)
        for (size_t j = 0; j < bt.strat.size(); ++j) out->strat_totals[j] = (accumulate ? out->strat_totals[j] : 0) + bt.strat[j];
}

static int prepare_outputs_on_device(avk_ctx *ctx, const avk_compare_out *out, u64 n_total, bool &want_seq, u64 &seq_bytes, bool &strata, bool &strat_dev) {
    const u64 n = ctx->n_regions, lo = ctx->lo;
    want_seq = out->seq_off && out->seq_len && out->seq_pool;
    seq_bytes = 0;
    ctx->seq_base = 0; ctx->strat_base = 0;
    if (want_seq) {
        for (u64 i = lo * 5; i < (lo + n) * 5; ++i) if (out->seq_off[i] > out->seq_off[i + 1]) { ctx->err = "seq_off is not monotone"; return AVK_ERR_INVALID; }
        ctx->seq_base = out->seq_off[lo * 5];
        seq_bytes = out->seq_off[(lo + n) * 5] - ctx->seq_base;
        UPLOAD(ctx->seq_off, out->seq_off + lo * 5, 8 * (n * 5 + 1));
        ENSURE(ctx->seq_len, 4 * 5 * n + 4);
        ENSURE(ctx->seq_pool, seq_bytes);
        CK(cudaMemsetAsync(ctx->seq_len.p, 0, 4 * 5 * n + 4, ctx->stream));
    }
    strata = strata_wanted(out);
    strat_dev = strata && !out->strat_off;
    if ((strat_dev || out->containment) && (ref_of(ctx)->st_n == 0 || (strat_dev && ref_of(ctx)->st_n != out->n_strata) || ref_of(ctx)->st_contigs != (u32)ref_of(ctx)->contig_lens.size())) {
        ctx->err = "the device containment lookup needs avk_set_stratifications (same number of strata as n_strata, contigs as the reference)";
        return AVK_ERR_INVALID;
    }
    if (strata && !strat_dev) {
        const u64 s0 = out->strat_off[lo], s1 = out->strat_off[lo + n];
        bool bad = s0 > s1 || (s1 > s0 && !out->strat_idx);
        for (u64 r = lo; r < lo + n && !bad; ++r) bad = out->strat_off[r] > out->strat_off[r + 1];
        for (u64 s = s0; s < s1 && !bad; ++s) bad = out->strat_idx[s] >= out->n_strata;
        if (bad) { ctx->err = "strat_off / strat_idx are inconsistent (not monotone, or a stratum index >= n_strata)"; return AVK_ERR_INVALID; }
        ctx->strat_base = s0;
        UPLOAD(ctx->strat_off, out->strat_off + lo, 8 * (n + 1));
        UPLOAD(ctx->strat_idx, out->strat_idx + s0, 4 * (s1 - s0));
    }
    (void)n_total;
    return AVK_OK;
}

static inline double host_ms() { return std::chrono::duration<double, std::milli>(std::chrono::steady_clock::now().time_since_epoch()).count(); }
struct BinPending {
    CompareRun R;
    bool want_seq = false, strata = false;
    u64 seq_bytes = 0;
};
static int bin_enqueue(avk_ctx *ctx, const avk_region_batch *batch, u64 lo, u64 hi, const avk_compare_cfg *cfg, avk_compare_out *out, BinPending &P) {
    CK(cudaSetDevice(ctx->device));
    const bool timing = getenv("AVK_TIMING") != nullptr;
    const double t0 = timing ? host_ms() : 0;
    BinScan sc;
    int rc = bin_range(ctx, batch, lo, hi, sc);
    if (rc != AVK_OK) return rc;
// ... 433 lines not shown
        ctx->launches += 12;
    } else {
        CK(cudaMemsetAsync(ctx->var_off.p, 0, 8, ctx->stream));
    }
    CK(cudaGetLastError());
    u64 kept_bytes = 0;
    if (nvalid) {
        u32 last[2] = {0, 0};
        CK(cudaMemcpyAsync(&last[0], (u32 *)ctx->aoff.p + (nvalid - 1), 4, cudaMemcpyDeviceToHost, ctx->stream));
        CK(cudaMemcpyAsync(&last[1], (u32 *)vend + (nvalid - 1), 4, cudaMemcpyDeviceToHost, ctx->stream));
        CK(cudaStreamSynchronize(ctx->stream));
        kept_bytes = (u64)last[0] + last[1];
    }
    CK(cudaStreamSynchronize(ctx->stream));
    ctx->n_regions = n; ctx->n_variants = nvalid; ctx->n_inputs = (u32)K; ctx->max_allele = mx; ctx->pool_len = kept_bytes; ctx->pool_bytes = kept_bytes;
    ctx->have_batch = ctx->ids_resident = true;
    *n_regions_out = n; *n_variants_out = nvalid;
    return AVK_OK;
}

extern "C" int avk_regions_download(avk_ctx *ctx, avk_region_batch *out) {
    if (!ctx || !out) return AVK_ERR_INVALID;
    if (!ctx->have_batch || ctx->lo != 0 || ctx->v_base != 0) { ctx->err = "avk_regions_download: no device-built batch is resident"; return AVK_ERR_INVALID; }
    CK(cudaSetDevice(ctx->device));
    const u64 n = ctx->n_regions, nv = ctx->n_variants, K = ctx->n_inputs;
    avk_variant_table &t = out->variants;
#define RBDL(dst, buf, bytes) do { if ((bytes) && (dst)) CK(cudaMemcpyAsync((void *)(dst), (buf).p, (bytes), cudaMemcpyDeviceToHost, ctx->stream)); } while (0)
    RBDL(out->region_id, ctx->region_id, 8 * n); RBDL(out->contig, ctx->contig, 4 * n); RBDL(out->start, ctx->start, 4 * n); RBDL(out->end, ctx->end, 4 * n);
    RBDL(out->var_off, ctx->var_off, 8 * (n * K + 1));
    RBDL(t.position, ctx->pos, 4 * nv); RBDL(t.variant_type, ctx->vtype, nv); RBDL(t.zygosity, ctx->zyg, nv); RBDL(t.raw_allele_space, ctx->raw, 4 * nv);
    RBDL(t.allele_off, ctx->aoff, 4 * nv); RBDL(t.a0_len, ctx->l0, 4 * nv); RBDL(t.a1_len, ctx->l1, 4 * nv); RBDL(t.allele_pool, ctx->pool, ctx->pool_bytes);
#undef RBDL
    CK(cudaStreamSynchronize(ctx->stream));
    out->n_regions = n; out->n_inputs = (uint32_t)K; t.n_variants = nv; t.allele_pool_len = ctx->pool_bytes;
    return AVK_OK;
}

extern "C" int avk_compare_upload_range(avk_ctx *ctx, const avk_region_batch *batch, uint64_t lo, uint64_t hi) {
    if (!ctx) return AVK_ERR_INVALID;
    CK(cudaSetDevice(ctx->device));
    int rc = validate_batch(ctx, batch, true);
    if (rc != AVK_OK) return rc;
    if (lo > hi || hi > batch->n_regions) { ctx->err = "region range outside the batch"; return AVK_ERR_INVALID; }
    BinScan sc;
    rc = bin_range(ctx, batch, lo, hi, sc);
    if (rc != AVK_OK) return rc;
    rc = upload_batch(ctx, batch, sc);
    if (rc != AVK_OK) return rc;
    ctx->seq_base = 0; ctx->strat_base = 0;
    CK(cudaStreamSynchronize(ctx->stream));
    return AVK_OK;
}

extern "C" int avk_compare_upload(avk_ctx *ctx, const avk_region_batch *batch) {
    if (!ctx) return AVK_ERR_INVALID;
    if (!batch) { ctx->err = "null batch"; return AVK_ERR_INVALID; }
    return avk_compare_upload_range(ctx, batch, 0, batch->n_regions);
}

extern "C" int avk_compare_run_resident(avk_ctx *ctx, const avk_compare_cfg *cfg) {
    if (!ctx) return AVK_ERR_INVALID;
    if (!cfg || !ctx->have_batch || ctx->n_inputs != 2) { ctx->err = "no resident compare batch"; return AVK_ERR_INVALID; }
    CK(cudaSetDevice(ctx->device));
    CompareRun R;
    int rc = compare_launch(ctx, cfg, false, (cfg->flags & AVK_CMP_KEEP_REGION_ROWS) != 0, false, 0, false, false, R);
    if (rc != AVK_OK) return rc;
    rc = compare_finish(ctx, R, nullptr);
    if (rc != AVK_OK) return rc;
    return fetch_timings(ctx);
}

extern "C" int avk_compare_download(avk_ctx *ctx, avk_compare_out *out) {
    if (!ctx) return AVK_ERR_INVALID;
    if (!out || !ctx->have_batch || !ctx->have_result) { ctx->err = "no compare result is resident (run avk_compare_run_resident first)"; return AVK_ERR_INVALID; }
    CK(cudaSetDevice(ctx->device));
    int rc = download_compare_async(ctx, out, false, 0);
    if (rc != AVK_OK) return rc;
    CK(cudaStreamSynchronize(ctx->stream));
    BinTotals bt;
    rc = collect_totals(ctx, out, false, bt);
    if (rc != AVK_OK) return rc;
    store_totals(out, bt, false, false);
    return AVK_OK;
}

extern "C" int avk_compare_result_device(avk_ctx *ctx, avk_compare_dev_view *v) {
    if (!ctx || !v) return AVK_ERR_INVALID;
    if (!ctx->have_batch || !ctx->have_result) { ctx->err = "no compare result is resident"; return AVK_ERR_INVALID; }
    v->lo = ctx->lo; v->n_regions = ctx->n_regions; v->v_base = ctx->v_base; v->n_variants = ctx->n_variants;
    v->status = ctx->status.p; v->ed1 = ctx->ed1.p; v->ed2 = ctx->ed2.p; v->type_mask = ctx->type_mask.p;
    v->var_expected = ctx->vexp.p; v->var_observed = ctx->vobs.p; v->var_class = ctx->vcls.p; v->totals = ctx->totals.p;
    return AVK_OK;
}

extern "C" int avk_int_peak(avk_ctx *ctx, double *ops_per_s) {
    if (!ctx || !ops_per_s) return AVK_ERR_INVALID;
    CK(cudaSetDevice(ctx->device));
    ENSURE(ctx->counters, 64);
    const int iters = 1 << 13, blocks = ctx->sm_count * 16, threads = 256;
    float best = 1e30f;
    for (int rep = 0; rep < 4; ++rep) {
        CK(cudaEventRecord(ctx->ev[0], ctx->stream));
        k_int_peak<<<blocks, threads, 0, ctx->stream>>>(iters, (int *)ctx->counters.p);
        CK(cudaEventRecord(ctx->ev[1], ctx->stream));
        CK(cudaEventSynchronize(ctx->ev[1]));
        float ms = 0;
        cudaEventElapsedTime(&ms, ctx->ev[0], ctx->ev[1]);
        if (rep > 0 && ms < best) best = ms;
    }
    ctx->launches += 4;
    CK(cudaGetLastError());
    *ops_per_s = (double)blocks * threads * (double)iters * 8.0 * 3.0 / (best * 1e-3);
    return AVK_OK;
}

extern "C" int avk_last_timings(avk_ctx *ctx, float *ms5) {
    if (!ctx || !ms5) return AVK_ERR_INVALID;
    memcpy(ms5, ctx->last_ms, sizeof(ctx->last_ms));
    return AVK_OK;
}
extern "C" int avk_last_tier_overflow(avk_ctx *ctx, uint32_t *out3) {
    if (!ctx || !out3) return AVK_ERR_INVALID;
    for (int i = 0; i < 3; ++i) out3[i] = ctx->tier_fail[i];
    return AVK_OK;
}
extern "C" int avk_last_tier_ms(avk_ctx *ctx, float *out3) {
    if (!ctx || !out3) return AVK_ERR_INVALID;
    for (int i = 0; i < 3; ++i) out3[i] = ctx->tier_ms[i];
    return AVK_OK;
}
extern "C" int avk_last_work(avk_ctx *ctx, avk_work_counters *out) {
    if (!ctx || !out) return AVK_ERR_INVALID;
    *out = ctx->last_work;
    return AVK_OK;
}

static int merge_bin(avk_ctx *ctx, const avk_region_batch *batch, u64 lo, u64 hi, const avk_merge_cfg *cfg, avk_merge_out *out) {
    CK(cudaSetDevice(ctx->device));
    BinScan sc;
    int rc = bin_range(ctx, batch, lo, hi, sc);
    if (rc != AVK_OK) return rc;
    rc = upload_batch(ctx, batch, sc);
    if (rc != AVK_OK) return rc;
    const u64 n = ctx->n_regions;
    const u32 K = ctx->n_inputs;
    ENSURE(ctx->status, 4 * n); ENSURE(ctx->m_cls, n); ENSURE(ctx->m_nidx, n); ENSURE(ctx->m_idx, n * K);
    ENSURE(ctx->counters, 64); ENSURE(ctx->work_ctr, 64);
    CK(cudaMemsetAsync(ctx->work_ctr.p, 0, 64, ctx->stream));
    DevBatch db = dev_batch(ctx);
    DevMergeOut mo;
    mo.status = (int *)ctx->status.p; mo.cls = (u8 *)ctx->m_cls.p; mo.n_idx = (u8 *)ctx->m_nidx.p; mo.idx = (u8 *)ctx->m_idx.p;
    avk_merge_cfg c = *cfg;
    CK(cudaEventRecord(ctx->ev[0], ctx->stream));
    rc = run_alt_ed(ctx, db);
    if (rc != AVK_OK) return rc;
    CK(cudaEventRecord(ctx->ev[1], ctx->stream));
    const int sm = ctx->sm_count;
    const int INF = 0x7fffffff;
    const u64 pairs = (u64)K * (K - 1) / 2, max_tasks = n * pairs;
    if (max_tasks >= 0xffffffffull || n >= (1ull << 47)) { ctx->err = "avk_merge_batch: too many pair tasks"; return AVK_ERR_INVALID; }
    ENSURE(ctx->m_rows, 4 * n * K); ENSURE(ctx->m_perr, 4 * n); ENSURE(ctx->m_tasks, 8 * max_tasks);
    MergeWork mw;
    mw.rows = (u32 *)ctx->m_rows.p; mw.pair_err = (u32 *)ctx->m_perr.p; mw.tasks = (u64 *)ctx->m_tasks.p; mw.task_ctr = nullptr;
    const std::vector<Stage> stages = {
        {MODE_FUSED, true, 3, 8192, sm * 3, 8, -1, 0, 0, 0, 1, 0, 0, INF},
        {MODE_FUSED, true, 1, 27648, sm, 8, 0, 1, 3, 1, 4, 0, 0, INF},
        {MODE_FUSED, false, 1, 2LL << 20, sm, 8, 1, 4, 5, 0, 6, 0, 0, INF},
    };
    const unsigned cgrid = (unsigned)std::min<u64>((u64)sm * 8, (n + 7) / 8);
    rc = run_stages(ctx, std::max<u64>(max_tasks, 1), stages, [&](u32 *ctrs) {
        mw.task_ctr = ctrs + 20;
        if (n) k_merge_front<<<cgrid, 256, 0, ctx->stream>>>(db, mo, c, mw, n);
        ctx->launches += 1;
    }, 20, [&](const Stage &st, const TierArgs &a, int ctas, cudaStream_t strm) {
        if (st.smem && st.min_ctas == 3) launch_merge_pairs<true, 3>(db, c, a, mw, ctas, st.warps, strm);
        else if (st.smem) launch_merge_pairs<true, 1>(db, c, a, mw, ctas, st.warps, strm);
        else launch_merge_pairs<false, 1>(db, c, a, mw, ctas, st.warps, strm);
    });
    if (rc != AVK_OK) return rc;
    if (n) {
        k_merge_classify<<<cgrid, 256, 0, ctx->stream>>>(db, mo, c, mw, n);
        ctx->launches += 1;
        CK(cudaGetLastError());
    }
    if (rc != AVK_OK) return rc;
    CK(cudaEventRecord(ctx->ev[2], ctx->stream));
    CK(cudaEventRecord(ctx->ev[3], ctx->stream));
    CK(cudaEventRecord(ctx->ev[4], ctx->stream));
    const cudaStream_t ds = ctx->stream;
    DL(out->status + lo, ctx->status, 4 * n);
    DL(out->classification ? out->classification + lo : nullptr, ctx->m_cls, n);
    DL(out->n_indices ? out->n_indices + lo : nullptr, ctx->m_nidx, n);
    DL(out->indices ? out->indices + lo * K : nullptr, ctx->m_idx, n * K);
    CK(cudaMemcpyAsync(ctx->h_pin + 128, ctx->work_ctr.p, 40, cudaMemcpyDeviceToHost, ctx->stream));
    CK(cudaEventRecord(ctx->ev_done, ctx->stream));
    CK(cudaStreamSynchronize(ctx->stream));
    return fetch_timings(ctx);
}

extern "C" int avk_merge_batch(avk_ctx *ctx, const avk_region_batch *batch, const avk_merge_cfg *cfg, avk_merge_out *out) {
    if (!ctx) return AVK_ERR_INVALID;
    if (!cfg || !out || !out->status) { ctx->err = "null cfg/out/status"; return AVK_ERR_INVALID; }
    int rc = validate_batch(ctx, batch, false);
    if (rc != AVK_OK) return rc;
    return merge_bin(ctx, batch, 0, batch->n_regions, cfg, out);
}

extern "C" int avk_merge_batch_multi(avk_ctx *const *ctxs, uint32_t n_ctx, const avk_region_batch *batch,
                                     const avk_merge_cfg *cfg, avk_merge_out *out) {
    if (!ctxs || n_ctx == 0 || !ctxs[0]) return AVK_ERR_INVALID;
    avk_ctx *ctx = ctxs[0];
    if (!cfg || !out || !out->status) { ctx->err = "null cfg/out/status"; return AVK_ERR_INVALID; }
    int rc = validate_batch(ctx, batch, false);
    if (rc != AVK_OK) return rc;
    std::vector<u64> cuts(n_ctx + 1);
    avk_partition_regions(batch, n_ctx, cuts.data());
    std::vector<int> rcs(n_ctx, AVK_OK);
    std::vector<std::thread> th;
    for (uint32_t k = 0; k < n_ctx; ++k)
        th.emplace_back([&, k]() { rcs[k] = ctxs[k] ? merge_bin(ctxs[k], batch, cuts[k], cuts[k + 1], cfg, out) : AVK_ERR_INVALID; });
    for (auto &t : th) t.join();
    for (uint32_t k = 0; k < n_ctx; ++k)
        if (rcs[k] != AVK_OK) { if (k && ctxs[k]) ctx->err = "device " + std::to_string(k) + ": " + ctxs[k]->err; return rcs[k]; }
    return AVK_OK;
}


extern "C" int avk_wfa_ed_batch(avk_ctx *ctx, uint64_t n_pairs, const uint8_t *pool, uint64_t pool_len, const uint64_t *a_off,
                                const uint32_t *a_len, const uint64_t *b_off, const uint32_t *b_len, uint32_t *ed_out) {
    if (!ctx) return AVK_ERR_INVALID;
    if (n_pairs && (!pool || !a_off || !a_len || !b_off || !b_len || !ed_out)) { ctx->err = "null argument"; return AVK_ERR_INVALID; }
    if (n_pairs >= (1ull << 32) - 1) { ctx->err = "too many pairs"; return AVK_ERR_INVALID; }
    CK(cudaSetDevice(ctx->device));
    if (n_pairs == 0) return AVK_OK;
    u32 mx = 1;
    for (u64 i = 0; i < n_pairs; ++i) {
        if (a_off[i] + a_len[i] > pool_len || b_off[i] + b_len[i] > pool_len) { ctx->err = "pair outside pool"; return AVK_ERR_INVALID; }
        mx = std::max(mx, std::max(a_len[i], b_len[i]));
    }
    UPLOAD(ctx->pair_pool, pool, pool_len);
    UPLOAD(ctx->pair_a_off, a_off, 8 * n_pairs);
    UPLOAD(ctx->pair_b_off, b_off, 8 * n_pairs);
    UPLOAD(ctx->pair_a_len, a_len, 4 * n_pairs);
    UPLOAD(ctx->pair_b_len, b_len, 4 * n_pairs);
    ENSURE(ctx->pair_ed, 4 * n_pairs);
    ENSURE(ctx->counters, 64); ENSURE(ctx->work_ctr, 64);
    CK(cudaMemsetAsync(ctx->counters.p, 0, 64, ctx->stream));
    CK(cudaMemsetAsync(ctx->work_ctr.p, 0, 64, ctx->stream));
    const int scratch_ints = (2 * (int)mx + 8 + 3) / 4 * 4;
    int warps = (int)std::min<u64>((u64)ctx->sm_count * 32, (n_pairs + 7) / 8 * 8);
    warps = (warps + 7) / 8 * 8;
    const int ctas = (int)std::min<u64>((u64)ctx->sm_count, n_pairs);
    ENSURE(ctx->scratch, (size_t)(warps + ctas) * ((size_t)scratch_ints * 4 + ARENA_HDR));
    ENSURE(ctx->fail_a, 4 * n_pairs); ENSURE(ctx->fail_b, 4 * n_pairs);
    u32 *ctrs = (u32 *)ctx->counters.p;
    const int cap_ints = ctx->coop_cap_ints;
    CK(cudaEventRecord(ctx->ev[0], ctx->stream));
    k_wfa_split<<<(unsigned)((n_pairs + 255) / 256), 256, 0, ctx->stream>>>(n_pairs, (const u32 *)ctx->pair_a_len.p, (const u32 *)ctx->pair_b_len.p, 512u,
                                                                          (u32)(8 * cap_ints), (u32 *)ctx->fail_a.p, ctrs + 2, (u32 *)ctx->fail_b.p, ctrs + 3);
    CK(cudaEventRecord(ctx->ev[1], ctx->stream));
    k_wfa_ed_cta<<<ctas, COOP_THREADS, COOP_JOB_BYTES + 2 * sizeof(int) * (size_t)cap_ints, ctx->stream>>>(
        (const u32 *)ctx->fail_b.p, ctrs + 3, (const u8 *)ctx->pair_pool.p, (const u64 *)ctx->pair_a_off.p, (const u32 *)ctx->pair_a_len.p,
        (const u64 *)ctx->pair_b_off.p, (const u32 *)ctx->pair_b_len.p, (u32 *)ctx->pair_ed.p,
        (u8 *)ctx->scratch.p + (size_t)warps * ((size_t)scratch_ints * 4 + ARENA_HDR), scratch_ints, cap_ints, ctrs + 1, (unsigned long long *)ctx->work_ctr.p);
    k_wfa_ed<<<warps / 8, 256, 0, ctx->stream>>>((const u32 *)ctx->fail_a.p, ctrs + 2, (const u8 *)ctx->pair_pool.p, (const u64 *)ctx->pair_a_off.p,
                                                  (const u32 *)ctx->pair_a_len.p, (const u64 *)ctx->pair_b_off.p,
                                                  (const u32 *)ctx->pair_b_len.p, (u32 *)ctx->pair_ed.p, (u8 *)ctx->scratch.p,
                                                  scratch_ints, ctrs, (unsigned long long *)ctx->work_ctr.p);
    ctx->launches += 2;
    ctx->launches += 1;
    CK(cudaGetLastError());
    CK(cudaEventRecord(ctx->ev[2], ctx->stream));
    CK(cudaEventRecord(ctx->ev[3], ctx->stream));
    CK(cudaEventRecord(ctx->ev[4], ctx->stream));
    ctx->have_result = false;
    CK(cudaMemcpyAsync(ed_out, ctx->pair_ed.p, 4 * n_pairs, cudaMemcpyDeviceToHost, ctx->stream));
    CK(cudaMemcpyAsync(ctx->h_pin + 128, ctx->work_ctr.p, 40, cudaMemcpyDeviceToHost, ctx->stream));
    CK(cudaEventRecord(ctx->ev_done, ctx->stream));
    CK(cudaStreamSynchronize(ctx->stream));
    return fetch_timings(ctx);
}

extern "C" int avk_compare_seq_offsets(const avk_region_batch *b, uint64_t *seq_off, uint64_t *pool_len) {
    if (!b || !seq_off || b->n_inputs != 2) return AVK_ERR_INVALID;
    u64 off = 0;
    for (u64 r = 0; r < b->n_regions; ++r) {
        const u64 win = b->end[r] > b->start[r] ? b->end[r] - b->start[r] : 0;
        u64 alt[2] = {0, 0};
        for (int k = 0; k < 2; ++k)
            for (u64 v = b->var_off[r * 2 + k]; v < b->var_off[r * 2 + k + 1]; ++v) alt[k] += b->variants.a1_len[v];
        const u64 sizes[5] = {win, win + alt[0], win + alt[0], win + alt[1], win + alt[1]};
        for (int s = 0; s < 5; ++s) { seq_off[r * 5 + s] = off; off += sizes[s]; }
    }
    seq_off[b->n_regions * 5] = off;
    if (pool_len) *pool_len = off;
    return AVK_OK;
}

static int copy_text(const std::string &txt, char *buf, uint64_t cap, uint64_t *len) {
    if (len) *len = txt.size();
    if (!buf) return AVK_OK;
    if (cap < txt.size()) return AVK_ERR_INVALID;
    memcpy(buf, txt.data(), txt.size());
    return AVK_OK;
}
extern "C" int avk_summary_write(const uint64_t *totals, const uint8_t *metrics, uint32_t n_metrics, const char *compare_label, const char *region_label,
                                 int csv, int header, char *buf, uint64_t cap, uint64_t *len) {
// ... 562 lines not shown
```

Measured before the change: 264.6 million.

## Classify simple regions before digest prep and restrict alt-ed and prep to the rest

```diff
diff --git a/aardvark_b200/csrc/avk_lib.cu b/aardvark_b200/csrc/avk_lib.cu
--- a/aardvark_b200/csrc/avk_lib.cu
+++ b/aardvark_b200/csrc/avk_lib.cu
@@ -59,42 +59,95 @@
     return v;
 }
 
+__device__ __forceinline__ u32 alt_ed_coop(const DevBatch &b, u64 vv, u64 hdr, int scratch_ints) {
+    const int l0 = (int)b.l0[vv], l1 = (int)b.l1[vv];
+    const u8 *a0 = b.pool + b.aoff[vv];
+    const u8 *a1 = a0 + l0;
+    int ed;
+    const int mn = min(l0, l1);
+    if (mn == 0) ed = max(l0, l1);
+    else if (2 * max(l0, l1) + 3 > scratch_ints) ed = 0;
+    else {
+        const int p = raw_lcp<false>((u64)(uintptr_t)a0, (u64)(uintptr_t)a1, mn);
+        if (p == mn) ed = max(l0, l1) - mn;
+        else {
+            ed = wfa_ed_warp<false>(plain_seq(a0, l0), plain_seq(a1, l1), hdr + ARENA_HDR, (scratch_ints - 3) / 2, hdr);
+            if (ed < 0) ed = 0;
+        }
+    }
+    return (u32)ed;
+}
+
+__device__ __forceinline__ void alt_ed_span(const DevBatch &b, u64 first, u64 end, u64 step, u32 *alt_ed, u64 hdr, int scratch_ints) {
+    const int lane = lane_id();
+    for (u64 base = first; base < end; base += step) {
+        const u64 v = base + lane;
+        bool coop = false;
+        if (v < end) {
+            const u32 l0 = b.l0[v], l1 = b.l1[v];
+            if (l0 == 1 && l1 == 1) alt_ed[v] = (b.pool[b.aoff[v]] != b.pool[b.aoff[v] + 1]) ? 1u : 0u;
+            else coop = true;
+        }
+        unsigned m = __ballot_sync(AVK_FULL, coop);
+        while (m) {
+            const int src = __ffs(m) - 1;
+            m &= m - 1;
+            const u32 ed = alt_ed_coop(b, base + src, hdr, scratch_ints);
+            if (lane == 0) alt_ed[base + src] = ed;
+        }
+    }
+}
+
 __global__ void __launch_bounds__(256) k_alt_ed(DevBatch b, u64 v_base, u64 n_variants, u32 *alt_ed, u8 *scratch, int scratch_ints,
                                                 unsigned long long *work_out) {
+    const u64 warp = ((u64)blockIdx.x * blockDim.x + threadIdx.x) >> 5;
+    const u64 n_warps = ((u64)gridDim.x * blockDim.x) >> 5;
+    const u64 hdr = (u64)(uintptr_t)(scratch + warp * ((u64)scratch_ints * 4 + ARENA_HDR));
+    clear_work<false>(hdr);
+    alt_ed_span(b, v_base + warp * 32, v_base + n_variants, n_warps * 32, alt_ed, hdr, scratch_ints);
+    flush_work<false>(hdr, work_out);
+}
+
+__global__ void __launch_bounds__(256) k_alt_ed_list(DevBatch b, const u32 *list, const u32 *n_list, u32 *alt_ed, u8 *scratch, int scratch_ints,
+                                                     unsigned long long *work_out) {
     const int lane = lane_id();
     const u64 warp = ((u64)blockIdx.x * blockDim.x + threadIdx.x) >> 5;
     const u64 n_warps = ((u64)gridDim.x * blockDim.x) >> 5;
     const u64 hdr = (u64)(uintptr_t)(scratch + warp * ((u64)scratch_ints * 4 + ARENA_HDR));
     clear_work<false>(hdr);
-    for (u64 base = v_base + warp * 32; base < v_base + n_variants; base += n_warps * 32) {
-        const u64 v = base + lane;
-        bool coop = false;
-        if (v < v_base + n_variants) {
-            const u32 l0 = b.l0[v], l1 = b.l1[v];
-            if (l0 == 1 && l1 == 1) alt_ed[v] = (b.pool[b.aoff[v]] != b.pool[b.aoff[v] + 1]) ? 1u : 0u;
-            else coop = true;
-        }
-        unsigned m = __ballot_sync(AVK_FULL, coop);
+    const u64 n = *n_list;
+    for (u64 base = warp * 32; base < n; base += n_warps * 32) {
+        u64 v = 0, ve = 0;
+        if (base + lane < n) {
+            const u64 r = list[base + lane];
+            v = b.var_off[r * 2]; ve = b.var_off[r * 2 + 2];
+        }
+        const bool wide = ve - v > 32;
+        const u64 w0 = v, w1 = ve;
+        if (wide) v = ve;
+        for (;;) {
+            bool coop = false;
+            for (; v < ve; ++v) {
+                const u32 l0 = b.l0[v], l1 = b.l1[v];
+                if (l0 != 1 || l1 != 1) { coop = true; break; }
+                alt_ed[v] = (b.pool[b.aoff[v]] != b.pool[b.aoff[v] + 1]) ? 1u : 0u;
+            }
+            unsigned m = __ballot_sync(AVK_FULL, coop);
+            if (!m) break;
+            while (m) {
+                const int src = __ffs(m) - 1;
+                m &= m - 1;
+                const u64 vv = __shfl_sync(AVK_FULL, v, src);
+                const u32 ed = alt_ed_coop(b, vv, hdr, scratch_ints);
+                if (lane == 0) alt_ed[vv] = ed;
+            }
+            if (coop) ++v;
+        }
+        unsigned m = __ballot_sync(AVK_FULL, wide);
         while (m) {
             const int src = __ffs(m) - 1;
             m &= m - 1;
-            const u64 vv = base + src;
-            const int l0 = (int)b.l0[vv], l1 = (int)b.l1[vv];
-            const u8 *a0 = b.pool + b.aoff[vv];
-            const u8 *a1 = a0 + l0;
-            int ed;
-            const int mn = min(l0, l1);
-            if (mn == 0) ed = max(l0, l1);
-            else if (2 * max(l0, l1) + 3 > scratch_ints) ed = 0;
-            else {
-                const int p = raw_lcp<false>((u64)(uintptr_t)a0, (u64)(uintptr_t)a1, mn);
-                if (p == mn) ed = max(l0, l1) - mn;
-                else {
-                    ed = wfa_ed_warp<false>(plain_seq(a0, l0), plain_seq(a1, l1), hdr + ARENA_HDR, (scratch_ints - 3) / 2, hdr);
-                    if (ed < 0) ed = 0;
-                }
-            }
-            if (lane == 0) alt_ed[vv] = (u32)ed;
+            alt_ed_span(b, __shfl_sync(AVK_FULL, w0, src), __shfl_sync(AVK_FULL, w1, src), 32, alt_ed, hdr, scratch_ints);
         }
     }
     flush_work<false>(hdr, work_out);
@@ -173,23 +226,19 @@
     if (cta) list_cta[atomicAdd(n_cta, 1u)] = (u32)p; else list_warp[atomicAdd(n_warp, 1u)] = (u32)p;
 }
 
-__global__ void __launch_bounds__(256) k_prep_size(DevBatch b, u64 n, u64 *sizes) {
-    const u64 r = (u64)blockIdx.x * blockDim.x + threadIdx.x;
-    if (r > n) return;
-    if (r == n) { sizes[r] = 0; return; }
-    const u64 v0 = b.var_off[r * 2], v1 = b.var_off[r * 2 + 2];
+__device__ __forceinline__ u64 digest_bytes(const DevBatch &b, u64 v0, u64 v1) {
     u64 alle = 0;
     for (u64 v = v0; v < v1; ++v) alle += (u64)min(b.l0[v], 1u << 24) + (u64)min(b.l1[v], 1u << 24);
-    sizes[r] = (PH_SIZE + VI_SIZE * (v1 - v0) + alle + 16 + 15) & ~15ull;
-}
-
-__global__ void __launch_bounds__(256) k_prep_fill(DevBatch b, u64 n_all, const u64 *offs, u8 *digest, const u32 *list, const u32 *n_list) {
+    return (PH_SIZE + VI_SIZE * (v1 - v0) + alle + 16 + 15) & ~15ull;
+}
+
+__global__ void __launch_bounds__(256) k_prep_fill(DevBatch b, const u64 *offs, u8 *digest, const u32 *list, const u32 *n_list) {
     const int lane = lane_id();
     const u64 warp = ((u64)blockIdx.x * blockDim.x + threadIdx.x) >> 5;
     const u64 n_warps = ((u64)gridDim.x * blockDim.x) >> 5;
-    const u64 n = list ? (u64)*n_list : n_all;
+    const u64 n = *n_list;
     for (u64 ri = warp; ri < n; ri += n_warps) {
-        const u64 r = list ? (u64)list[ri] : ri;
+        const u64 r = list[ri];
         u8 *dig = digest + offs[r];
         int *hdr = (int *)dig;
         const long long start = b.start[r], end = b.end[r];
@@ -269,9 +318,7 @@
 }
 
 enum { PREP_SMALL_N = 12 };
-__global__ void __launch_bounds__(256) k_prep_fill_small(DevBatch b, u64 n, const u64 *offs, u8 *digest, u32 *big, u32 *big_ctr) {
-    const u64 r = (u64)blockIdx.x * blockDim.x + threadIdx.x;
-    if (r >= n) return;
+__device__ __forceinline__ void prep_fill_one(const DevBatch &b, u64 r, const u64 *offs, u8 *digest, u32 *big, u32 *big_ctr) {
     const u64 v0 = b.var_off[r * 2], vq = b.var_off[r * 2 + 1], v1 = b.var_off[r * 2 + 2];
     const int nT = (int)(vq - v0), nQ = (int)(v1 - vq), N = nT + nQ;
     if (N > PREP_SMALL_N) { big[atomicAdd(big_ctr, 1u)] = (u32)r; return; }
@@ -318,6 +365,12 @@
     h4[2] = make_uint4((u32)__popc(seen), st[0], st[1], st[2]);
     h4[3] = make_uint4(0, 0, 0, 0);
 }
+__global__ void __launch_bounds__(256) k_prep_fill_small(DevBatch b, const u32 *list, const u32 *n_list, const u64 *offs, u8 *digest, u32 *big,
+                                                         u32 *big_ctr) {
+    const u64 n = *n_list;
+    for (u64 i = (u64)blockIdx.x * blockDim.x + threadIdx.x; i < n; i += (u64)gridDim.x * blockDim.x)
+        prep_fill_one(b, list[i], offs, digest, big, big_ctr);
+}
 
 __device__ __forceinline__ void zero_region_outputs(const DevBatch &b, const DevCompareOut &out, u64 r, bool metrics_only) {
     const int lane = lane_id();
@@ -334,94 +387,83 @@
     __syncwarp();
 }
 
-__global__ void __launch_bounds__(256) k_compare_simple(DevBatch b, DevCompareOut out, avk_compare_cfg cfg, u64 n, u32 *work_list,
-                                                        u32 *work_ctr, u32 *dense, u32 *dense_ctr, int dense_n, u64 *work_key) {
+__device__ __forceinline__ u32 alt_ed_short(const u8 *a, u32 l0, u32 l1) {
+    const u8 c = l0 == 1 ? a[0] : a[l0];
+    const u8 *s = l0 == 1 ? a + 1 : a;
+    const u32 L = l0 == 1 ? l1 : l0;
+    bool hit = false;
+    for (u32 k = 0; k < L; ++k) hit = hit || s[k] == c;
+    return hit ? L - 1 : L;
+}
+
+__global__ void __launch_bounds__(256, 2) k_compare_simple(DevBatch b, DevCompareOut out, avk_compare_cfg cfg, u64 n, u64 *sizes, u32 *solve,
+                                                        u32 *solve_ctr) {
     const int lane = lane_id();
     const u64 warp = ((u64)blockIdx.x * blockDim.x + threadIdx.x) >> 5;
     const u64 n_warps = ((u64)gridDim.x * blockDim.x) >> 5;
     const bool enabled = !cfg.enable_exact_shortcut && !(out.seq_off && cfg.enable_sequences) && cfg.max_branch_factor >= 4;
     const u32 supported = (1u << AVK_VT_SNV) | (1u << AVK_VT_INSERTION) | (1u << AVK_VT_DELETION) | (1u << AVK_VT_INDEL) |
                           (1u << AVK_VT_TR_CONTRACTION) | (1u << AVK_VT_TR_EXPANSION) | (1u << AVK_VT_SV_DELETION) | (1u << AVK_VT_SV_INSERTION);
+    if (blockIdx.x == 0 && threadIdx.x == 0) sizes[n] = 0;
     for (u64 base = warp * 32; base < n; base += n_warps * 32) {
         const u64 r = base + lane;
         bool simple = false;
-        int nvar = 0, npairs = 0;
+        int npairs = 0;
         u32 gv[4] = {0, 0, 0, 0}, cp[2] = {0, 0}, vtype = 0;
         u64 s_c = 0, s_wT = 0, s_wQ = 0, s_X = 0, s_rT = 0, s_rQ = 0;
+        u64 v0 = 0, v1 = 0;
         if (r < n) {
-            const u8 *dig = b.digest + b.digest_off[r];
-            const int4 h = *(const int4 *)dig;
+            v0 = b.var_off[r * 2];
+            const u64 vq = b.var_off[r * 2 + 1];
+            v1 = b.var_off[r * 2 + 2];
             const u32 c = b.contig[r];
-            nvar = h.x == AVK_ST_OK ? h.y : 0;
-            const int M = (h.y == 2 && h.z == 1 && h.w == 1) ? 1 : ((h.y == 4 && h.z == 2 && h.w == 2) ? 2 : 0);
-            if (enabled && h.x == AVK_ST_OK && M && (M == 1 || cfg.max_branch_factor >= 16) && c < b.n_contigs && b.start[r] <= b.end[r] &&
-                (u64)b.end[r] <= b.contig_len[c] && b.end[r] <= 0x7fff0000u) {
-                const u8 *alle = dig + PH_SIZE + 2 * M * VI_SIZE;
+            const int M = (vq - v0 == 1 && v1 - vq == 1) ? 1 : ((vq - v0 == 2 && v1 - vq == 2) ? 2 : 0);
+            const long long start = b.start[r], end = b.end[r];
+            if (enabled && M && (M == 1 || cfg.max_branch_factor >= 16) && c < b.n_contigs && start <= end &&
+                (u64)end <= b.contig_len[c] && end <= 0x7fff0000LL) {
                 bool ok = true;
                 u32 prev_pos = 0;
-                for (int m = 0; m < M && ok; ++m) {
-                    const u8 *rt = dig + PH_SIZE + 2 * m * VI_SIZE, *rq = rt + VI_SIZE;
-                    const uint4 t0 = *(const uint4 *)rt, t1 = *(const uint4 *)(rt + 16), q0 = *(const uint4 *)rq, q1 = *(const uint4 *)(rq + 16);
-                    const u32 zT = (t1.w >> 8) & 0xff, zQ = (q1.w >> 8) & 0xff;
+#pragma unroll
+                for (int m = 0; m < 2; ++m) {
+                    if (m >= M || !ok) break;
+                    const u64 t = v0 + m, q = vq + m;
+                    const u32 p = b.pos[t], l0 = b.l0[t], l1 = b.l1[t], ty = b.vtype[t], zT = b.zyg[t], zQ = b.zyg[q];
                     const u32 cT = zT == AVK_ZYG_HOM_ALT ? 2u : (zT >= AVK_ZYG_UNPHASED_HET ? 1u : 0u);
                     const u32 cQ = zQ == AVK_ZYG_HOM_ALT ? 2u : (zQ >= AVK_ZYG_UNPHASED_HET ? 1u : 0u);
-                    const u32 ty = t1.w & 0xffu;
-                    ok = (t1.w & 0x10000u) && !(q1.w & 0x10000u) && ty == (q1.w & 0xffu) && ((supported >> ty) & 1u) && t0.x == q0.x &&
-                         t0.y == q0.y && t0.z == q0.z && (t0.y == 1 || t0.z == 1) && t0.y + t0.z <= 64 && cT != 0 && cT == cQ;
-                    if (M == 2) ok = ok && t0.y == 1 && t0.z == 1 && ty == AVK_VT_SNV && (m == 0 || t0.x > prev_pos);
+                    ok = l0 != 0 && l1 != 0 && ty < AVK_N_VARIANT_TYPES && zT <= AVK_ZYG_HOM_ALT && zQ <= AVK_ZYG_HOM_ALT &&
+                         (long long)p >= start && (long long)p + l0 <= end;
+                    ok = ok && b.pos[q] == p && b.l0[q] == l0 && b.l1[q] == l1 && b.vtype[q] == ty && ((supported >> ty) & 1u) &&
+                         (l0 == 1 || l1 == 1) && (u64)l0 + l1 <= 64 && cT != 0 && cT == cQ;
+                    if (M == 2) ok = ok && l0 == 1 && l1 == 1 && ty == AVK_VT_SNV && (m == 0 || p > prev_pos);
                     if (!ok) break;
-                    const u8 *aT = alle + t0.w + t0.y, *aQ = alle + q0.w + q0.y;
-                    for (u32 k = 0; k < t0.z; ++k) ok = ok && aT[k] == aQ[k];
-                    const bool anchored = aT[0] == b.contig_ptr[c][t0.x];
+                    const u8 *rT = b.pool + b.aoff[t], *rQ = b.pool + b.aoff[q];
+                    for (u32 k = 0; k < l1; ++k) ok = ok && rT[l0 + k] == rQ[l0 + k];
+                    const bool anchored = rT[l0] == b.contig_ptr[c][p];
                     u32 X = 0;
-                    if (t0.y == 1 && t0.z == 1) X = anchored ? 0u : 1u;
-                    else if (anchored) X = (t0.y == 1 ? t0.z : t0.y) - 1u;
-                    ok = ok && X != 0 && t1.y >= X && q1.y >= X;
-                    gv[2 * m] = t1.z; gv[2 * m + 1] = q1.z; cp[m] = cT; vtype = ty; prev_pos = t0.x;
-                    s_c += cT; s_wT += (u64)cT * t1.x; s_wQ += (u64)cT * q1.x; s_X += (u64)cT * X; s_rT += (u64)cT * t1.y; s_rQ += (u64)cT * q1.y;
+                    if (l0 == 1 && l1 == 1) X = anchored ? 0u : 1u;
+                    else if (anchored) X = (l0 == 1 ? l1 : l0) - 1u;
+                    const u32 rawT = b.raw[t], rawQ = b.raw[q];
+                    ok = ok && X != 0 && rawT >= X && rawQ >= X;
+                    if (!ok) break;
+                    gv[2 * m] = (u32)t; gv[2 * m + 1] = (u32)q; cp[m] = cT; vtype = ty; prev_pos = p;
+                    s_c += cT; s_wT += (u64)cT * alt_ed_short(rT, l0, l1); s_wQ += (u64)cT * alt_ed_short(rQ, l0, l1);
+                    s_X += (u64)cT * X; s_rT += (u64)cT * rawT; s_rQ += (u64)cT * rawQ;
                 }
                 simple = ok;
                 npairs = M;
             }
-        }
-        const bool is_dense = r < n && !simple && nvar >= dense_n;
-        const u32 rest = __ballot_sync(AVK_FULL, r < n && !simple && !is_dense);
-        const u32 dn = __ballot_sync(AVK_FULL, is_dense);
-        u32 pos0 = 0, pos1 = 0;
-        if (lane == 0 && rest) pos0 = atomicAdd(work_ctr, (u32)__popc(rest));
-        if (lane == 0 && dn) pos1 = atomicAdd(dense_ctr, (u32)__popc(dn));
+            sizes[r] = simple ? 0 : digest_bytes(b, v0, v1);
+        }
+        const u32 rest = __ballot_sync(AVK_FULL, r < n && !simple);
+        u32 pos0 = 0;
+        if (lane == 0 && rest) pos0 = atomicAdd(solve_ctr, (u32)__popc(rest));
         pos0 = __shfl_sync(AVK_FULL, pos0, 0);
-        pos1 = __shfl_sync(AVK_FULL, pos1, 0);
-        if (r < n && !simple && !is_dense) {
-            const u32 slot_ = pos0 + __popc(rest & ((1u << lane) - 1));
-            work_list[slot_] = (u32)r;
-            if (work_key) {
-                u64 key = 0;
-                const int *dh = (const int *)(b.digest + b.digest_off[r]);
-                const u32 edb = (u32)min(max(dh[PH_B0 / 4], 0), 16);
-                const u32 wgt = (u32)max(nvar, 1) * (edb + 1u) * (edb + 1u);
-                const u32 heavy = min(15u, (u32)(31 - __clz((int)max(wgt, 1u))));
-                if (nvar > 0 && nvar <= 9) {
-                    const u8 *recs = b.digest + b.digest_off[r] + PH_SIZE;
-                    u32 prev = 0xffffffffu;
-                    for (int oi = 0; oi < nvar; ++oi) {
-                        const uint4 a = *(const uint4 *)(recs + (size_t)VI_SIZE * oi);
-                        const u32 f = *(const u32 *)(recs + (size_t)VI_SIZE * oi + VI_FLAGS);
-                        const u32 lc = (a.y == 1 && a.z == 1) ? 0u : (a.y == 1 ? 1u : (a.z == 1 ? 2u : 3u));
-                        const u32 code = ((f >> 16) & 1u) | ((((f >> 8) & 0xffu) & 3u) << 1) | ((a.x == prev ? 1u : 0u) << 3) | (lc << 4);
-                        key = (key << 6) | code;
-                        prev = a.x;
-                    }
-                    key |= (u64)nvar << 54;
-                } else key = (u64)min(nvar, 15) << 54;
-                key |= (u64)(15u - heavy) << 58;
-                work_key[slot_] = key;
-            }
-        }
-        if (is_dense) dense[pos1 + __popc(dn & ((1u << lane) - 1))] = (u32)r;
+        if (r < n && !simple) solve[pos0 + __popc(rest & ((1u << lane) - 1))] = (u32)r;
         if (simple) {
             out.status[r] = AVK_ST_OK; out.ed1[r] = 0; out.ed2[r] = 0; out.type_mask[r] = (uint16_t)supported;
-            for (int m = 0; m < npairs; ++m) {
+#pragma unroll
+            for (int m = 0; m < 2; ++m) {
+                if (m >= npairs) break;
                 out.vexp[gv[2 * m]] = (u8)cp[m]; out.vobs[gv[2 * m]] = (u8)cp[m]; out.vcls[gv[2 * m]] = AVK_CLASS_TP;
                 out.vexp[gv[2 * m + 1]] = (u8)cp[m]; out.vobs[gv[2 * m + 1]] = (u8)cp[m]; out.vcls[gv[2 * m + 1]] = AVK_CLASS_TP;
             }
@@ -479,6 +521,54 @@
                 dst[i] = v;
             }
         }
+    }
+}
+
+__global__ void __launch_bounds__(256) k_route(DevBatch b, const u32 *solve, const u32 *solve_ctr, u32 *work_list, u32 *work_ctr, u32 *dense,
+                                               u32 *dense_ctr, int dense_n, u64 *work_key) {
+    const int lane = lane_id();
+    const u64 warp = ((u64)blockIdx.x * blockDim.x + threadIdx.x) >> 5;
+    const u64 n_warps = ((u64)gridDim.x * blockDim.x) >> 5;
+    const u64 n = *solve_ctr;
+    for (u64 base = warp * 32; base < n; base += n_warps * 32) {
+        const bool live = base + lane < n;
+        const u32 r = live ? solve[base + lane] : 0u;
+        const int *dh = (const int *)(b.digest + b.digest_off[r]);
+        const int nvar = live && dh[PH_STATUS / 4] == AVK_ST_OK ? dh[PH_N / 4] : 0;
+        const bool is_dense = live && nvar >= dense_n;
+        const u32 rest = __ballot_sync(AVK_FULL, live && !is_dense);
+        const u32 dn = __ballot_sync(AVK_FULL, is_dense);
+        u32 pos0 = 0, pos1 = 0;
+        if (lane == 0 && rest) pos0 = atomicAdd(work_ctr, (u32)__popc(rest));
+        if (lane == 0 && dn) pos1 = atomicAdd(dense_ctr, (u32)__popc(dn));
+        pos0 = __shfl_sync(AVK_FULL, pos0, 0);
+        pos1 = __shfl_sync(AVK_FULL, pos1, 0);
+        if (live && !is_dense) {
+            const u32 slot_ = pos0 + __popc(rest & ((1u << lane) - 1));
+            work_list[slot_] = r;
+            if (work_key) {
+                u64 key = 0;
+                const u32 edb = (u32)min(max(dh[PH_B0 / 4], 0), 16);
+                const u32 wgt = (u32)max(nvar, 1) * (edb + 1u) * (edb + 1u);
+                const u32 heavy = min(15u, (u32)(31 - __clz((int)max(wgt, 1u))));
+                if (nvar > 0 && nvar <= 9) {
+                    const u8 *recs = (const u8 *)dh + PH_SIZE;
+                    u32 prev = 0xffffffffu;
+                    for (int oi = 0; oi < nvar; ++oi) {
+                        const uint4 a = *(const uint4 *)(recs + (size_t)VI_SIZE * oi);
+                        const u32 f = *(const u32 *)(recs + (size_t)VI_SIZE * oi + VI_FLAGS);
+                        const u32 lc = (a.y == 1 && a.z == 1) ? 0u : (a.y == 1 ? 1u : (a.z == 1 ? 2u : 3u));
+                        const u32 code = ((f >> 16) & 1u) | ((((f >> 8) & 0xffu) & 3u) << 1) | ((a.x == prev ? 1u : 0u) << 3) | (lc << 4);
+                        key = (key << 6) | code;
+                        prev = a.x;
+                    }
+                    key |= (u64)nvar << 54;
+                } else key = (u64)min(nvar, 15) << 54;
+                key |= (u64)(15u - heavy) << 58;
+                work_key[slot_] = key;
+            }
+        }
+        if (is_dense) dense[pos1 + __popc(dn & ((1u << lane) - 1))] = r;
     }
 }
 
@@ -1124,7 +1214,7 @@
     DevBuf region_id, contig, start, end, var_off, pos, vtype, zyg, raw, aoff, l0, l1, pool, alt_ed;
     DevBuf status, ed1, ed2, region_metrics, type_mask, vexp, vobs, vcls, totals, tot_slots, strat_off, strat_idx, strat_totals,
         seq_off, seq_len, seq_pool, m_cls, m_nidx, m_idx, m_rows, m_perr, m_tasks;
-    DevBuf digest, digest_sizes, digest_offs, scan_tmp, blobs, scratch, arena, arena2, counters, fail_a, fail_b, fail_c, fail_d, fail_h, fail_w, fail_x, fail_t, fail_s, shape_key, work_ctr, pair_a_off, pair_b_off, pair_a_len, pair_b_len, pair_ed, pair_pool;
+    DevBuf digest, digest_sizes, digest_offs, scan_tmp, blobs, scratch, arena, arena2, counters, solve_list, fail_a, fail_b, fail_c, fail_d, fail_h, fail_w, fail_x, fail_t, fail_s, shape_key, work_ctr, pair_a_off, pair_b_off, pair_a_len, pair_b_len, pair_ed, pair_pool;
     DevBuf rb[24];
     DevBuf st_off, st_first, st_pmax, st_mask;
     u32 st_n = 0, st_contigs = 0;
@@ -1319,7 +1409,7 @@
                       &ctx->pos, &ctx->vtype, &ctx->zyg, &ctx->raw, &ctx->aoff, &ctx->l0, &ctx->l1, &ctx->pool, &ctx->alt_ed,
                       &ctx->status, &ctx->ed1, &ctx->ed2, &ctx->region_metrics, &ctx->type_mask, &ctx->vexp, &ctx->vobs, &ctx->vcls,
                       &ctx->totals, &ctx->tot_slots, &ctx->strat_off, &ctx->strat_idx, &ctx->strat_totals, &ctx->seq_off, &ctx->seq_len, &ctx->seq_pool,
-                      &ctx->m_cls, &ctx->m_nidx, &ctx->m_idx, &ctx->m_rows, &ctx->m_perr, &ctx->m_tasks, &ctx->digest, &ctx->digest_sizes, &ctx->digest_offs, &ctx->scan_tmp, &ctx->blobs, &ctx->scratch, &ctx->arena, &ctx->arena2, &ctx->counters, &ctx->fail_a, &ctx->fail_b, &ctx->fail_c, &ctx->fail_d, &ctx->fail_h, &ctx->fail_w, &ctx->fail_x, &ctx->fail_t, &ctx->fail_s, &ctx->shape_key, &ctx->dense_blobs, &ctx->dense_blobs2, &ctx->spec_prof,
+                      &ctx->m_cls, &ctx->m_nidx, &ctx->m_idx, &ctx->m_rows, &ctx->m_perr, &ctx->m_tasks, &ctx->digest, &ctx->digest_sizes, &ctx->digest_offs, &ctx->scan_tmp, &ctx->blobs, &ctx->scratch, &ctx->arena, &ctx->arena2, &ctx->counters, &ctx->solve_list, &ctx->fail_a, &ctx->fail_b, &ctx->fail_c, &ctx->fail_d, &ctx->fail_h, &ctx->fail_w, &ctx->fail_x, &ctx->fail_t, &ctx->fail_s, &ctx->shape_key, &ctx->dense_blobs, &ctx->dense_blobs2, &ctx->spec_prof,
                       &ctx->work_ctr, &ctx->pair_a_off, &ctx->pair_b_off, &ctx->pair_a_len, &ctx->pair_b_len, &ctx->pair_ed, &ctx->pair_pool};
     for (DevBuf *b : bufs) if (b->p) cudaFree(b->p);
     for (DevBuf &b : ctx->rb) if (b.p) cudaFree(b.p);
@@ -1521,14 +1611,16 @@
     return d;
 }
 
-static int run_alt_ed(avk_ctx *ctx, const DevBatch &db) {
+static int run_alt_ed(avk_ctx *ctx, const DevBatch &db, const u32 *list, const u32 *n_list) {
     if (ctx->n_variants == 0) return AVK_OK;
     const int blocks = ctx->sm_count * 4, threads = 256;
     const int warps = blocks * threads / 32;
     const int scratch_ints = (2 * (int)ctx->max_allele + 8 + 3) / 4 * 4;
     ENSURE(ctx->scratch, (size_t)warps * ((size_t)scratch_ints * 4 + ARENA_HDR));
-    k_alt_ed<<<blocks, threads, 0, ctx->stream>>>(db, ctx->v_base, ctx->n_variants, biased<u32>(ctx->alt_ed, ctx->v_base), (u8 *)ctx->scratch.p,
-                                                   scratch_ints, (unsigned long long *)ctx->work_ctr.p);
+    u32 *alt_ed = biased<u32>(ctx->alt_ed, ctx->v_base);
+    unsigned long long *work = (unsigned long long *)ctx->work_ctr.p;
+    if (list) k_alt_ed_list<<<blocks, threads, 0, ctx->stream>>>(db, list, n_list, alt_ed, (u8 *)ctx->scratch.p, scratch_ints, work);
+    else k_alt_ed<<<blocks, threads, 0, ctx->stream>>>(db, ctx->v_base, ctx->n_variants, alt_ed, (u8 *)ctx->scratch.p, scratch_ints, work);
     ctx->launches += 1;
     CK(cudaGetLastError());
     return AVK_OK;
@@ -1643,26 +1735,6 @@
     k_merge_pairs<SMEM, MIN_CTAS><<<ctas, 32 * warps, smem, strm>>>(db, c, a, w);
 }
 
-static int run_prepare(avk_ctx *ctx, const DevBatch &db) {
-    const u64 n = ctx->n_regions;
-    if (n == 0) return AVK_OK;
-    u64 *sizes = (u64 *)ctx->digest_sizes.p, *offs = (u64 *)ctx->digest_offs.p;
-    k_prep_size<<<(unsigned)((n + 1 + 255) / 256), 256, 0, ctx->stream>>>(db, n, sizes);
-    size_t tmp_bytes = 0;
-    cub::DeviceScan::ExclusiveSum(nullptr, tmp_bytes, sizes, offs, (int)(n + 1), ctx->stream);
-    ENSURE(ctx->scan_tmp, tmp_bytes);
-    cub::DeviceScan::ExclusiveSum(ctx->scan_tmp.p, tmp_bytes, sizes, offs, (int)(n + 1), ctx->stream);
-    ENSURE(ctx->fail_a, 4 * n);
-    ENSURE(ctx->counters, 256);
-    u32 *big_ctr = (u32 *)ctx->counters.p + 40;
-    CK(cudaMemsetAsync(big_ctr, 0, 4, ctx->stream));
-    k_prep_fill_small<<<(unsigned)((n + 255) / 256), 256, 0, ctx->stream>>>(db, n, offs, (u8 *)ctx->digest.p, (u32 *)ctx->fail_a.p, big_ctr);
-    k_prep_fill<<<ctx->sm_count * 2, 256, 0, ctx->stream>>>(db, n, offs, (u8 *)ctx->digest.p, (const u32 *)ctx->fail_a.p, big_ctr);
-    ctx->launches += 4;
-    CK(cudaGetLastError());
-    return AVK_OK;
-}
-
 static inline bool strata_wanted(const avk_compare_out *out) { return out->strat_totals && out->n_strata; }
 
 struct CompareRun {
@@ -1699,39 +1771,74 @@
     return a;
 }
 
-static int run_compare_pipeline(avk_ctx *ctx, const CompareRun &R) {
+struct Routing {
+    bool thread_stage;
+    int dense_n;
+    bool sort_shapes;
+};
+static Routing routing(const avk_ctx *ctx) {
+    const u64 n = ctx->n_regions;
+    Routing rt;
+    rt.thread_stage = ctx->use_thread_stage && n >= (ctx->many_in_flight ? ctx->thread_min_regions_lanes : ctx->thread_min_regions);
+    rt.dense_n = ctx->dense_n ? ctx->dense_n : (rt.thread_stage ? 10 : (n >= 250000 ? 8 : 6));
+    rt.sort_shapes = rt.thread_stage && ctx->sort_shapes;
+    return rt;
+}
+
+static int run_front_end(avk_ctx *ctx, const CompareRun &R, const Routing &rt) {
+    const u64 n = ctx->n_regions;
+    ENSURE(ctx->counters, 256);
+    u32 *ctrs = (u32 *)ctx->counters.p;
+    CK(cudaMemsetAsync(ctrs, 0, 256, ctx->stream));
+    if (n == 0) return AVK_OK;
+    const int sm = ctx->sm_count;
+    ENSURE(ctx->solve_list, 4 * n); ENSURE(ctx->fail_a, 4 * n); ENSURE(ctx->fail_h, 4 * n); ENSURE(ctx->fail_x, 4 * n);
+    u64 *keys = nullptr;
+    if (rt.sort_shapes) {
+        ENSURE(ctx->shape_key, 16 * n);
+        ENSURE(ctx->fail_s, 4 * n);
+        keys = (u64 *)ctx->shape_key.p;
+    }
+    u32 *LS = (u32 *)ctx->solve_list.p, *LW = (u32 *)ctx->fail_h.p, *LX = (u32 *)ctx->fail_x.p;
+    u64 *sizes = (u64 *)ctx->digest_sizes.p, *offs = (u64 *)ctx->digest_offs.p;
+    k_compare_simple<<<sm * 8, 256, 0, ctx->stream>>>(R.db, R.out, R.cfg, n, sizes, LS, ctrs + 41);
+    size_t tmp_bytes = 0;
+    cub::DeviceScan::ExclusiveSum(nullptr, tmp_bytes, sizes, offs, (int)(n + 1), ctx->stream);
+    ENSURE(ctx->scan_tmp, tmp_bytes);
+    cub::DeviceScan::ExclusiveSum(ctx->scan_tmp.p, tmp_bytes, sizes, offs, (int)(n + 1), ctx->stream);
+    const int rc = run_alt_ed(ctx, R.db, LS, ctrs + 41);
+    if (rc != AVK_OK) return rc;
+    k_prep_fill_small<<<(unsigned)std::min<u64>((n + 255) / 256, (u64)sm * 8), 256, 0, ctx->stream>>>(R.db, LS, ctrs + 41, offs, (u8 *)ctx->digest.p,
+                                                                                                      (u32 *)ctx->fail_a.p, ctrs + 40);
+    k_prep_fill<<<sm * 2, 256, 0, ctx->stream>>>(R.db, offs, (u8 *)ctx->digest.p, (const u32 *)ctx->fail_a.p, ctrs + 40);
+    if (keys) CK(cudaMemsetAsync(keys, 0xff, 8 * n, ctx->stream));
+    k_route<<<sm * 8, 256, 0, ctx->stream>>>(R.db, LS, ctrs + 41, LW, ctrs + 12, LX, ctrs + 17, rt.dense_n, keys);
+    ctx->launches += 5;
+    if (keys) {
+        size_t need = 0;
+        cub::DeviceRadixSort::SortPairs(nullptr, need, keys, keys + n, LW, (u32 *)ctx->fail_s.p, (int)n, 0, 64, ctx->stream);
+        ENSURE(ctx->scan_tmp, need);
+        cub::DeviceRadixSort::SortPairs(ctx->scan_tmp.p, need, keys, keys + n, LW, (u32 *)ctx->fail_s.p, (int)n, 0, 64, ctx->stream);
+        ctx->launches += 1;
+    }
+    CK(cudaGetLastError());
+    return AVK_OK;
+}
+
+static int run_compare_pipeline(avk_ctx *ctx, const CompareRun &R, const Routing &rt) {
     const u64 n = ctx->n_regions;
     if (n == 0) return AVK_OK;
     const int sm = ctx->sm_count;
     ENSURE(ctx->fail_a, 4 * n); ENSURE(ctx->fail_b, 4 * n); ENSURE(ctx->fail_c, 4 * n); ENSURE(ctx->fail_d, 4 * n); ENSURE(ctx->fail_h, 4 * n); ENSURE(ctx->fail_w, 4 * n); ENSURE(ctx->fail_x, 4 * n); ENSURE(ctx->fail_t, 4 * n);
     ENSURE(ctx->counters, 256);
     ENSURE(ctx->blobs, (size_t)n * RB_SIZE);
-    u32 *ctrs = (u32 *)ctx->counters.p;
     u32 *LA = (u32 *)ctx->fail_a.p, *LB = (u32 *)ctx->fail_b.p, *LD = (u32 *)ctx->fail_d.p;
-    CK(cudaMemsetAsync(ctrs, 0, 256, ctx->stream));
     ENSURE(ctx->arena, (size_t)sm * 8 * (size_t)(2LL << 20));
     ENSURE(ctx->arena2, 2 * (size_t)sm * 8 * (size_t)(1u << 20));
     const Stage SEARCH = {MODE_SEARCH, true, 3, 8192, sm * 3, 8}, SCORE = {MODE_SCORE, true, 4, 5120, sm * 4, 8};
     const Stage S1 = {MODE_FUSED, true, 1, 27648, sm, 8}, G0 = {MODE_FUSED, false, 1, 2LL << 20, sm, 8};
     CK(cudaEventRecord(ctx->tev[0], ctx->stream));
     u32 *LW = (u32 *)ctx->fail_h.p, *LA2 = (u32 *)ctx->fail_w.p, *LX = (u32 *)ctx->fail_x.p;
-    const bool thread_stage = ctx->use_thread_stage && n >= (ctx->many_in_flight ? ctx->thread_min_regions_lanes : ctx->thread_min_regions);
-    const int dense_n = ctx->dense_n ? ctx->dense_n : (thread_stage ? 10 : (n >= 250000 ? 8 : 6));
-    u64 *keys = nullptr;
-    if (thread_stage && ctx->sort_shapes) {
-        ENSURE(ctx->shape_key, 16 * n);
-        ENSURE(ctx->fail_s, 4 * n);
-        keys = (u64 *)ctx->shape_key.p;
-        CK(cudaMemsetAsync(keys, 0xff, 8 * n, ctx->stream));
-    }
-    k_compare_simple<<<sm * 8, 256, 0, ctx->stream>>>(R.db, R.out, R.cfg, n, LW, ctrs + 12, LX, ctrs + 17, dense_n, keys);
-    if (keys) {
-        size_t need = 0;
-        cub::DeviceRadixSort::SortPairs(nullptr, need, keys, keys + n, LW, (u32 *)ctx->fail_s.p, (int)n, 0, 64, ctx->stream);
-        ENSURE(ctx->scan_tmp, need);
-        cub::DeviceRadixSort::SortPairs(ctx->scan_tmp.p, need, keys, keys + n, LW, (u32 *)ctx->fail_s.p, (int)n, 0, 64, ctx->stream);
-        ctx->launches += 1;
-    }
     const size_t spill_warp = 1u << 20, spill_half = (size_t)sm * 8 * spill_warp;
     const u32 dense_cap = (u32)std::min<u64>(n, std::max<u64>(65536, n / 16));
     auto spec_then_team = [&](const u32 *list, int in_ctr, int spec_ctr, int team_ctr, DevBuf &blobs, u8 *spill, cudaStream_t strm) -> int {
@@ -1756,9 +1863,9 @@
         if (rc != AVK_OK) return rc;
     }
     CK(cudaEventRecord(ctx->tev[1], ctx->stream));
-    if (thread_stage) {
+    if (rt.thread_stage) {
         u32 *LW2 = (u32 *)ctx->fail_t.p;
-        TierArgs a = tier_args(ctx, keys ? (const u32 *)ctx->fail_s.p : LW, 12, 19, LW2, 13, sizeof(avk_ts::Work), nullptr);
+        TierArgs a = tier_args(ctx, rt.sort_shapes ? (const u32 *)ctx->fail_s.p : LW, 12, 19, LW2, 13, sizeof(avk_ts::Work), nullptr);
         a.batch_min = ctx->thread_batch_min;
         a.pop_budget = ctx->thread_pop_budget ? ctx->thread_pop_budget : (n >= 2500000 ? 64 : (n >= 1200000 ? 48 : 32));
         k_compare_thread<<<(unsigned)std::min<u64>((u64)sm, (n + THREAD_TPB - 1) / THREAD_TPB), THREAD_TPB, THREAD_TPB * sizeof(avk_ts::Work), ctx->side[0]>>>(R.db, R.out, R.cfg, a);
@@ -1787,7 +1894,7 @@
         launch_stage(ctx, R, G0, a, G0.ctas, ctx->stream);
     }
     CK(cudaEventRecord(ctx->tev[3], ctx->stream));
-    ctx->launches += 3;
+    ctx->launches += 2;
     CK(cudaGetLastError());
     return AVK_OK;
 }
@@ -1884,10 +1991,9 @@
     R.want_contain = strat_dev || want_contain;
     ctx->have_result = false;
 
+    const Routing rt = routing(ctx);
     CK(cudaEventRecord(ctx->ev[0], ctx->stream));
-    int rc = run_alt_ed(ctx, R.db);
-    if (rc != AVK_OK) return rc;
-    rc = run_prepare(ctx, R.db);
+    int rc = run_front_end(ctx, R, rt);
     if (rc != AVK_OK) return rc;
     CK(cudaEventRecord(ctx->ev[1], ctx->stream));
     if (R.want_contain && n) {
@@ -1896,7 +2002,7 @@
                                                                               (const u32 *)so->st_first.p, (const u32 *)so->st_pmax.p, (u64 *)ctx->st_mask.p);
         ctx->launches += 1;
     }
-    rc = run_compare_pipeline(ctx, R);
+    rc = run_compare_pipeline(ctx, R, rt);
     if (rc != AVK_OK) return rc;
     CK(cudaEventRecord(ctx->ev[2], ctx->stream));
     CK(cudaEventRecord(ctx->ev[3], ctx->stream));
@@ -2636,7 +2742,7 @@
     mo.status = (int *)ctx->status.p; mo.cls = (u8 *)ctx->m_cls.p; mo.n_idx = (u8 *)ctx->m_nidx.p; mo.idx = (u8 *)ctx->m_idx.p;
     avk_merge_cfg c = *cfg;
     CK(cudaEventRecord(ctx->ev[0], ctx->stream));
-    rc = run_alt_ed(ctx, db);
+    rc = run_alt_ed(ctx, db, nullptr, nullptr);
     if (rc != AVK_OK) return rc;
     CK(cudaEventRecord(ctx->ev[1], ctx->stream));
     const int sm = ctx->sm_count;
```

Result: faster. 274.8 million (median of 6 runs) (+3.8%).
